# weiaicunzai/pytorch-camvid

Hardware: AMD Instinct MI355X
Metric: images/sec fwd+bwd UNet 3x360x480 bs=8 (higher is better)
Workload: dtype f32; 1 GPU; UNET(3,12) train fwd+bwd+CE, per-GPU batch 8 x 3x360x480 fp32 (BASELINE.json configs[1]); global_batch=8, parallelism=dp1

## Files before the change

### include/cvk.h

```cpp
#ifndef CVK_H
#define CVK_H

#include <stddef.h>
#include <stdint.h>

#ifdef __cplusplus
extern "C" {
#endif

#define CVK_VERSION 100
#define CVK_OK 0
#define CVK_EINVAL (-1)
#define CVK_EWORKSPACE (-2)
#define CVK_STAT_ROWS 64

typedef struct cvk_view {
    float*  ptr;
    int64_t sN, sY, sX;
} cvk_view;

typedef struct cvk_viewh {
    void*   ptr;
    int64_t sN, sY, sX;
} cvk_viewh;
// ... 122 lines not shown
int cvk_conv3x3_thin_fwd(const float* x, const float* w, const float* bias, float* y, float* stats, float* counts, int N, int H,
                         int W, int Cin_ld, int Cout, int ldy, void* stream);
int cvk_thin_wgrad_supported(int Cin, int Cin_ld, int Cout, int ld_dy);
size_t cvk_conv3x3_thin_wgrad_workspace_bytes(int N, int H, int W, int Cin_ld, int Cout);
int cvk_conv3x3_thin_wgrad(const float* x, const float* dy, float* dw, int N, int H, int W, int Cin, int Cin_ld, int Cout,
                           int ld_dy, void* workspace, size_t workspace_bytes, void* stream);

size_t cvk_conv3x3_wgradp_workspace_bytes(int N, int H, int W, int Cin_pad, int Cout);
int cvk_conv3x3_wgradp(const float* x, const float* dy, const float* E6_pre, float* dw, int N, int H, int W, int Cin, int Cin_pad,
                       int Cout, int ld_dy, void* workspace, size_t workspace_bytes, void* stream);
long cvk_wgradp_plane_rows(int N, int H, int W);
int cvk_wgradp_planes(const float* t, int ld, float* planes, int N, int H, int W, int C, int is_dy, void* stream);
size_t cvk_wgradp_gemm_workspace_bytes(int N, int H, int W, int Cin_pad, int Cout);
int cvk_wgradp_gemm(const float* E6, const float* V6, float* dw, int N, int H, int W, int Cin, int Cin_pad, int Cout, void* workspace,
                    size_t workspace_bytes, void* stream);
int cvk_wgradp_zero_pads(float* planes, int N, int H, int W, int C, void* stream);
int cvk_wgradp_zero_pads_sm(float* planes, int N, int H, int W, int C, void* stream);
int cvk_wgradp_planes_sm(const float* x, int ld, float* planes, int N, int H, int W, int C, void* stream);
int cvk_wgradp_gemm_sm(const float* E6, const float* V6sm, float* dw, int N, int H, int W, int Cin, int Cin_pad, int Cout, void* workspace,
                       size_t workspace_bytes, void* stream);
int cvk_wgradp_zero_pads4(float* planes, int N, int H, int W, int C, void* stream);
int cvk_bn_bwd_dx_e4p(cvk_view dout, const float* y, int ldy, const float* scale, const float* shift, const float* mean,
                      const float* rstd, const float* dgamma, const float* dbeta, float* dy, int ld_dy, float* E4p, float* part,
                      int N, int H, int W, int C, int use_batch_stats, void* stream);
int cvk_wgradp_dy_slack(int W);
int cvk_wgradp_gemm_sm_dy(const float* E4p, const float* dy, const float* V6sm, float* dw, int N, int H, int W, int Cin, int Cin_pad, int Cout,
                          void* workspace, size_t workspace_bytes, void* stream);
int cvk_wgradp_gemm_wg(const float* E6, const float* V6, float* dw, int N, int H, int W, int Cin, int Cin_pad, int Cout, void* workspace,
                       size_t workspace_bytes, int max_workgroups, void* stream);
int cvk_wgradp_gemm_sm_wg(const float* E6, const float* V6sm, float* dw, int N, int H, int W, int Cin, int Cin_pad, int Cout, void* workspace,
                          size_t workspace_bytes, int max_workgroups, void* stream);
int cvk_wgradp_gemm_sm_dy_wg(const float* E4p, const float* dy, const float* V6sm, float* dw, int N, int H, int W, int Cin, int Cin_pad, int Cout,
                             void* workspace, size_t workspace_bytes, int max_workgroups, void* stream);
void* cvk_side_begin(void* main_stream);
int cvk_side_join(void* main_stream);
long cvk_side_launches(void);
int cvk_bn_bwd_dx_e6(cvk_view dout, const float* y, int ldy, const float* scale, const float* shift, const float* mean,
                     const float* rstd, const float* dgamma, const float* dbeta, float* dy, int ld_dy, float* E6, float* part,
                     int N, int H, int W, int C, int use_batch_stats, void* stream);

size_t cvk_conv3x3_wgrad_wino4_workspace_bytes(int N, int H, int W, int Cin_pad, int Cout, int ld_dy);
int cvk_conv3x3_wgrad_wino4(const float* x, const float* dy, const float* E_pre, float* dw, int N, int H, int W, int Cin,
                            int Cin_pad, int Cout, int ld_dy, void* workspace, size_t workspace_bytes, void* stream);
int cvk_bn_bwd_e_blocks(int N, int H, int W);
int cvk_bn_bwd_dx_e(cvk_view dout, const float* y, int ldy, const float* scale, const float* shift, const float* mean,
                    const float* rstd, const float* dgamma, const float* dbeta, float* dy, int ld_dy, float* E, float* part,
                    int N, int H, int W, int C, int use_batch_stats, void* stream);

size_t cvk_conv3x3_wgrad_wino_workspace_bytes(int N, int H, int W, int Cin_pad, int Cout);
int cvk_conv3x3_wgrad_wino(const float* x, const float* dy, float* dw, int N, int H, int W, int Cin, int Cin_pad,
                           int Cout, int ld_dy, void* workspace, size_t workspace_bytes, void* stream);

size_t cvk_bn_finalize_workspace_bytes(int P, int C);
int cvk_bn_finalize(const float* stats, int P, int M, int C, const float* gamma, const float* beta,
                    float* mean, float* rstd, float* scale, float* shift,
                    float* running_mean, float* running_var, int64_t* num_batches_tracked,
                    float momentum, float eps, void* workspace, size_t workspace_bytes, void* stream);
int cvk_bn_eval_params(const float* gamma, const float* beta, const float* running_mean, const float* running_var,
                       float* mean, float* rstd, float* scale, float* shift, int C, float eps, void* stream);
int cvk_bn_relu_apply(const float* y, int ldy, const float* scale, const float* shift, cvk_view out,
                      int N, int H, int W, int C, void* stream);
int cvk_bn_relu_apply_pool(const float* y, int ldy, const float* scale, const float* shift, cvk_view out, float* pool,
                           unsigned char* code, int N, int H, int W, int C, void* stream);
int cvk_bn_bwd_blocks(int M);
int cvk_bn_bwd_reduce(cvk_view dout, const float* y, int ldy, const float* scale, const float* shift,
                      const float* mean, const float* rstd, float* part, int N, int H, int W, int C, void* stream);
int cvk_colsum_finalize(const float* part, int PB, int C, float* out0, float* out1, void* stream);
#define CVK_COLSUM_BATCH_MAX 64
typedef struct cvk_colsum_job { const float* part; float* out; int PB, C; } cvk_colsum_job;
int cvk_colsum_finalize_batch(const cvk_colsum_job* jobs, int n, void* stream);
int cvk_bn_relu_apply_amax(const float* y, int ldy, const float* scale, const float* shift, cvk_view out, int N, int H, int W, int C,
                           void* amax_block, void* stream);
int cvk_bn_relu_apply_pool_amax(const float* y, int ldy, const float* scale, const float* shift, cvk_view out, float* pool,
                                unsigned char* code, int N, int H, int W, int C, void* amax_out, void* amax_pool, void* stream);
int cvk_bn_bwd_dx_e_amax(int six, cvk_view dout, const float* y, int ldy, const float* scale, const float* shift, const float* mean,
                         const float* rstd, const float* dgamma, const float* dbeta, float* dy, int ld_dy, float* E, float* part, int N, int H,
                         int W, int C, int use_batch_stats, void* amax_block, void* stream);
int cvk_bn_bwd_dx_amax(cvk_view dout, const float* y, int ldy, const float* scale, const float* shift, const float* mean,
                       const float* rstd, const float* dgamma, const float* dbeta, float* dy, int ld_dy, float* dbias_part, int N,
                       int H, int W, int C, int use_batch_stats, void* amax_block, void* stream);
int cvk_bn_bwd_dx(cvk_view dout, const float* y, int ldy, const float* scale, const float* shift,
                  const float* mean, const float* rstd, const float* dgamma, const float* dbeta,
                  float* dy, int ld_dy, float* dbias_part, int N, int H, int W, int C, int use_batch_stats, void* stream);

int cvk_maxpool2x2_fwd(cvk_view x, float* out, uint8_t* code, int N, int H, int W, int C, void* stream);
int cvk_maxpool2x2_bwd(const float* dout, cvk_view x, const uint8_t* code, cvk_view dx, int accumulate,
                       int N, int H, int W, int C, void* stream);
int cvk_maxpool2x2_bwd_bnred_blocks(int N, int H, int W, int C);
int cvk_maxpool2x2_bwd_bnred(const float* dout, cvk_view x, const uint8_t* code, cvk_view dx, int accumulate, int N, int H, int W, int C,
                             const float* yP, int ldp, const float* scale, const float* shift, const float* mean, const float* rstd,
                             float* part, void* stream);
int cvk_maxunpool2x2_fwd(const float* v, const uint8_t* code, float* out, int N, int H, int W, int C, void* stream);
int cvk_maxunpool2x2_bwd(const float* dout, const uint8_t* code, float* dv, int N, int H, int W, int C, void* stream);
int cvk_pool_code_to_index(const uint8_t* code, int64_t* idx, int N, int H, int W, int C, void* stream);

int cvk_bilinear_up2_fwd(const float* x, float* out, int N, int H, int W, int C, void* stream);
int cvk_bilinear_up2_bwd(const float* dout, float* dx, int N, int H, int W, int C, void* stream);

int cvk_ce_blocks(int M);
int cvk_softmax_ce_fwd(const float* logits, int ld, const int64_t* target, float* part, float* loss,
                       int M, int C, int ignore_index, void* stream);
int cvk_softmax_ce_bwd(const float* logits, int ld, const int64_t* target, const float* loss3, const float* grad_out,
                       float scale, float* dlogits, int ld_d, int M, int C, int ignore_index, void* stream);

#define CVK_REDUCTION_NONE 0
#define CVK_REDUCTION_MEAN 1
#define CVK_REDUCTION_SUM 2
int cvk_ce_ex_part_floats(int M);
int cvk_softmax_ce_fwd_ex(const float* logits, int ld, const int64_t* target, const float* weight, float label_smoothing,
                          int reduction, float* part, float* loss, float* loss_px, int M, int C, int ignore_index, void* stream);
int cvk_softmax_ce_bwd_ex(const float* logits, int ld, const int64_t* target, const float* weight, float label_smoothing,
                          int reduction, const float* loss4, const float* grad_out, float scale, float* dlogits, int ld_d,
                          int M, int C, int ignore_index, void* stream);

#define CVK_DICE_PRESENT 0
#define CVK_DICE_ALL 1
int cvk_seg_loss_part_floats(int M, int C);
int cvk_seg_loss_record_floats(int C);
int cvk_seg_loss_fwd(const float* logits, int ld, const int64_t* target, const float* weight, float ce, float dice, float focal_gamma,
                     float dice_smooth, int dice_average, float* part, float* record, int M, int C, int ignore_index, void* stream);
int cvk_seg_loss_bwd(const float* logits, int ld, const int64_t* target, const float* weight, float ce, float dice, float focal_gamma,
                     const float* record, const float* grad_out, float scale, float* dlogits, int ld_d, int M, int C, int ignore_index,
                     void* stream);

int cvk_kd_loss_part_floats(int M);
int cvk_kd_loss_record_floats(void);
int cvk_kd_loss_fwd(const float* student, int ld_s, const float* teacher, int ld_t, const int64_t* target, const float* weight, float ce,
                    float kd, float tau, float t2, int distill_ignored, float* part, float* record, int M, int C, int ignore_index,
                    void* stream);
int cvk_kd_loss_bwd(const float* student, int ld_s, const float* teacher, int ld_t, const int64_t* target, const float* weight, float ce,
                    float kd, float tau, float t2, int distill_ignored, const float* record, const float* grad_out, float scale,
                    float* dlogits, int ld_d, int M, int C, int ignore_index, void* stream);

int cvk_ohem_scratch_bytes(int M);
int cvk_ohem_record_floats(void);
int cvk_ohem_ce_fwd(const float* logits, int ld, const int64_t* target, const float* weight, float loss_thresh, int min_kept,
                    void* scratch, float* record, float* loss_px, int M, int C, int ignore_index, void* stream);
int cvk_ohem_ce_bwd(const float* logits, int ld, const int64_t* target, const float* weight, const float* record,
                    const float* loss_px, const float* grad_out, float scale, float* dlogits, int ld_d, int M, int C, int ignore_index,
                    void* stream);

#define CVK_LOVASZ_PRESENT 0
#define CVK_LOVASZ_ALL 1
#define CVK_LOVASZ_DIGIT_BITS 8
#define CVK_LOVASZ_SORT_TILE 2048
int64_t cvk_lovasz_workspace_bytes(int M, int C, int segments);
int     cvk_lovasz_record_floats(void);
int64_t cvk_lovasz_sort_dest(int64_t seg_len, int64_t segment, int64_t digit_base, int64_t wg_base, int64_t rank);
int64_t cvk_lovasz_sort_count_index(int64_t work_groups, int64_t segment, int64_t digit, int64_t work_group);
int cvk_lovasz_softmax_fwd(const float* logits, int ld, const int64_t* target, const float* weight, float lovasz, float ce,
                           int classes_mode, int per_image, int N, int pixels_per_image, void* workspace, float* record, float* gmap,
                           int ld_g, int C, int ignore_index, void* stream);
int cvk_lovasz_softmax_bwd(const float* logits, int ld, const int64_t* target, const float* weight, float lovasz, float ce,
                           int per_image, int N, int pixels_per_image, const void* workspace, const float* record, const float* gmap,
                           int ld_g, const float* grad_out, float scale, float* dlogits, int ld_d, int C, int ignore_index,
                           void* stream);

int64_t cvk_edt_workspace_bytes(int N, int H, int W, int num_classes);
int cvk_edt_squared(const int64_t* labels, int N, int H, int W, int num_classes, int ignore_index, void* workspace, int32_t* to_class,
                    int32_t* to_other, void* stream);
int cvk_edt_signed(const int64_t* labels, int N, int H, int W, int num_classes, int ignore_index, void* workspace, float* phi,
                   void* stream);
int cvk_boundary_loss_part_floats(int M, int C);
int cvk_boundary_loss_record_floats(void);
int cvk_boundary_loss_fwd(const float* logits, int ld, const int64_t* target, const float* phi, const float* weight, const float* coef,
                          int want_boundary, int want_ce, unsigned class_mask, float* part, float* record, int M, int C,
// ... 208 lines not shown
```

### pytorch-camvid_amd/_lib.py

```python
import ctypes
import os
import subprocess
import threading

_HERE = os.path.dirname(os.path.abspath(__file__))
LIB_PATH = os.environ.get("CVK_LIB_PATH") or os.path.join(_HERE, "lib", "libcvk.so")
CSRC = os.path.join(_HERE, "csrc")
HEADER = os.path.join(os.path.dirname(_HERE), "include", "cvk.h")

CVK_STAT_ROWS = 64

c_f32p = ctypes.c_void_p
c_i64 = ctypes.c_int64
c_int = ctypes.c_int
c_size = ctypes.c_size_t
c_float = ctypes.c_float
c_vp = ctypes.c_void_p


class View(ctypes.Structure):
    _fields_ = [("ptr", ctypes.c_void_p), ("sN", ctypes.c_int64), ("sY", ctypes.c_int64), ("sX", ctypes.c_int64)]


class ViewH(ctypes.Structure):
# ... 62 lines not shown
    "cvk_side_begin": (c_vp, [c_vp]),
    "cvk_side_join": (c_int, [c_vp]),
    "cvk_side_launches": (ctypes.c_long, []),
    "cvk_conv3x3_wino4f_vplanes": (c_int, [c_vp, c_vp, c_vp, c_vp, c_vp, c_vp, c_vp, c_int, c_int, c_int, c_int, c_int, c_int, c_int, c_vp]),
    "cvk_bn_bwd_dx_e6": (c_int, [View, c_vp, c_int, c_vp, c_vp, c_vp, c_vp, c_vp, c_vp, c_vp, c_int, c_vp, c_vp,
                                 c_int, c_int, c_int, c_int, c_int, c_vp]),
    "cvk_w2d_tiles": (c_int, [c_int, c_int, c_int]),
    "cvk_w6_tiles": (c_int, [c_int, c_int, c_int]),
    "cvk_w6_stat_partials": (c_int, [c_int, c_int, c_int]),
    "cvk_conv3x3_w6_workspace_bytes": (c_size, [c_int, c_int, c_int, c_int, c_int]),
    "cvk_w6_weight_transform": (c_int, [c_vp, c_vp, c_int, c_int, c_vp]),
    "cvk_w6_weight_transform_dgrad": (c_int, [c_vp, c_vp, c_int, c_int, c_vp]),
    "cvk_w6_input_transform": (c_int, [c_vp, c_vp, c_int, c_int, c_int, c_int, c_vp]),
    "cvk_w6_gemm": (c_int, [c_vp, c_vp, c_vp, c_int, c_int, c_int, c_vp]),
    "cvk_w6_wgrad_ksplit": (c_int, [c_int, c_int, c_int]),
    "cvk_w6_dy_transform": (c_int, [c_vp, c_int, c_vp, c_int, c_int, c_int, c_int, c_vp]),
    "cvk_w6_gemm_tn": (c_int, [c_vp, c_vp, c_vp, c_int, c_int, c_int, c_vp]),
    "cvk_w6_wgrad_output": (c_int, [c_vp, c_vp, c_int, c_int, c_int, c_int, c_vp]),
    "cvk_w6_ksplit": (c_int, [c_int, c_int, c_int]),
    "cvk_w6_output": (c_int, [c_vp, c_vp, c_vp, c_vp, c_vp, c_int, c_int, c_int, c_int, c_int, c_int, c_vp]),
    "cvk_w2d_stat_partials": (c_int, [c_int, c_int, c_int]),
    "cvk_conv3x3_w2d_workspace_bytes": (c_size, [c_int, c_int, c_int, c_int, c_int]),
    "cvk_w2d_weight_transform": (c_int, [c_vp, c_vp, c_int, c_int, c_vp]),
    "cvk_w2d_weight_transform_dgrad": (c_int, [c_vp, c_vp, c_int, c_int, c_vp]),
    "cvk_w2d_input_transform": (c_int, [c_vp, c_vp, c_int, c_int, c_int, c_int, c_vp]),
    "cvk_w2d_gemm": (c_int, [c_vp, c_vp, c_vp, c_int, c_int, c_int, c_vp]),
    "cvk_conv3x3_wgrad_w2d_workspace_bytes": (c_size, [c_int, c_int, c_int, c_int, c_int]),
    "cvk_conv3x3_wgrad_w2d": (c_int, [c_vp, c_vp, c_vp, c_int, c_int, c_int, c_int, c_int, c_int, c_int, c_vp, c_size, c_vp]),
    "cvk_w2d_tpad": (c_int, [c_int]),
    "cvk_split3_rows_pad": (c_int, [c_int, c_int]),
    "cvk_split3_planes": (c_int, [c_vp, c_vp, c_int, c_int, c_int, c_int, c_vp]),
    "cvk_w2d_gemm_split3": (c_int, [c_vp, c_vp, c_vp, c_int, c_int, c_int, c_int, c_int, c_int, c_vp]),
    "cvk_w2d_input_transform_split3": (c_int, [c_int, c_vp, c_vp, c_int, c_int, c_int, c_int, c_vp]),
    "cvk_w2d_dy_transform_both_split3": (c_int, [c_int, c_vp, c_int, c_vp, c_vp, c_int, c_int, c_int, c_int, c_int, c_vp]),
    "cvk_w2d_weight_transform_split3": (c_int, [c_int, c_vp, c_vp, c_vp, c_int, c_int, c_int, c_vp]),
    "cvk_w2d_output_plain": (c_int, [c_int, c_vp, c_vp, c_vp, c_vp, c_vp, c_int, c_int, c_int, c_int, c_int, c_vp]),
    "cvk_w2d_gemm_tn_split3_ksplit": (c_int, [c_int, c_int, c_int, c_int]),
    "cvk_w2d_gemm_tn_split3": (c_int, [c_vp, c_vp, c_vp, c_int, c_int, c_int, c_int, c_vp]),
    "cvk_amax_block_words": (c_int, []),
    "cvk_amax_block_value": (ctypes.c_uint, [c_vp, c_int]),
    "cvk_absmax_f32": (c_int, [c_vp, ctypes.c_long, c_int, c_int, c_vp, c_vp]),
    "cvk_split_scale_exponent": (c_int, [c_int, c_int, c_int, ctypes.c_uint]),
    "cvk_split_planes": (c_int, [c_int, c_int, c_int, c_vp, c_vp, c_vp, c_int, c_int, c_int, c_int, c_vp]),
    "cvk_w2d_gemm_split": (c_int, [c_int, c_int, c_vp, c_vp, c_vp, c_vp, c_vp, c_int, c_int, c_int, c_int, c_int, c_int, c_vp]),
    "cvk_w2d_input_transform_split": (c_int, [c_int, c_int, c_vp, c_vp, c_vp, c_int, c_int, c_int, c_int, c_vp]),
    "cvk_w2d_dy_transform_both_split": (c_int, [c_int, c_int, c_vp, c_int, c_vp, c_vp, c_int, c_vp, c_int, c_int, c_int, c_int, c_vp]),
    "cvk_w2d_weight_transform_split": (c_int, [c_int, c_int, c_vp, c_vp, c_vp, c_int, c_int, c_int, c_vp]),
    "cvk_w2d_gemm_tn_split": (c_int, [c_int, c_int, c_vp, c_vp, c_vp, c_vp, c_vp, c_int, c_int, c_int, c_int, c_vp]),
    "cvk_w2d_wgrad_output_f": (c_int, [c_int, c_vp, c_vp, c_int, c_int, c_int, c_int, c_vp]),
    "cvk_w2d_wgrad_ksplit": (c_int, [c_int, c_int, c_int]),
    "cvk_w2d_dy_transform": (c_int, [c_vp, c_int, c_vp, c_int, c_int, c_int, c_int, c_vp]),
    "cvk_w2d_dy_transform_both": (c_int, [c_vp, c_int, c_vp, c_vp, c_int, c_int, c_int, c_int, c_vp]),
    "cvk_w6_dy_transform_both": (c_int, [c_vp, c_int, c_vp, c_vp, c_int, c_int, c_int, c_int, c_vp]),
    "cvk_w2d_gemm_tn": (c_int, [c_vp, c_vp, c_vp, c_int, c_int, c_int, c_vp]),
    "cvk_w2d_wgrad_output": (c_int, [c_vp, c_vp, c_int, c_int, c_int, c_int, c_vp]),
    "cvk_w2d_ksplit": (c_int, [c_int, c_int, c_int]),
    "cvk_w2d_output": (c_int, [c_vp, c_vp, c_vp, c_vp, c_vp, c_int, c_int, c_int, c_int, c_int, c_int, c_vp]),
    "cvk_conv3x3_w2d": (c_int, [c_vp, c_vp, c_vp, c_vp, c_vp, c_vp, c_int, c_int, c_int, c_int, c_int, c_int, c_vp, c_size, c_vp]),
    "cvk_conv3x3_wgrad_wino4_workspace_bytes": (c_size, [c_int, c_int, c_int, c_int, c_int, c_int]),
    "cvk_conv3x3_wgrad_wino4": (c_int, [c_vp, c_vp, c_vp, c_vp, c_int, c_int, c_int, c_int, c_int, c_int, c_int, c_vp, c_size, c_vp]),
    "cvk_bn_bwd_e_blocks": (c_int, [c_int, c_int, c_int]),
    "cvk_bn_bwd_dx_e": (c_int, [View, c_vp, c_int, c_vp, c_vp, c_vp, c_vp, c_vp, c_vp, c_vp, c_int, c_vp, c_vp,
                                c_int, c_int, c_int, c_int, c_int, c_vp]),
    "cvk_conv3x3_wgrad_wino_workspace_bytes": (c_size, [c_int, c_int, c_int, c_int, c_int]),
    "cvk_conv3x3_wgrad_wino": (c_int, [c_vp, c_vp, c_vp, c_int, c_int, c_int, c_int, c_int, c_int, c_int, c_vp, c_size, c_vp]),
    "cvk_bn_finalize_workspace_bytes": (c_size, [c_int, c_int]),
    "cvk_bn_finalize": (c_int, [c_vp, c_int, c_int, c_int, c_vp, c_vp, c_vp, c_vp, c_vp, c_vp, c_vp, c_vp, c_vp,
                                c_float, c_float, c_vp, c_size, c_vp]),
    "cvk_bn_eval_params": (c_int, [c_vp, c_vp, c_vp, c_vp, c_vp, c_vp, c_vp, c_vp, c_int, c_float, c_vp]),
    "cvk_bn_relu_apply": (c_int, [c_vp, c_int, c_vp, c_vp, View, c_int, c_int, c_int, c_int, c_vp]),
    "cvk_bn_relu_apply_pool": (c_int, [c_vp, c_int, c_vp, c_vp, View, c_vp, c_vp, c_int, c_int, c_int, c_int, c_vp]),
    "cvk_bn_bwd_blocks": (c_int, [c_int]),
    "cvk_bn_bwd_reduce": (c_int, [View, c_vp, c_int, c_vp, c_vp, c_vp, c_vp, c_vp, c_int, c_int, c_int, c_int, c_vp]),
    "cvk_colsum_finalize": (c_int, [c_vp, c_int, c_int, c_vp, c_vp, c_vp]),
    "cvk_colsum_finalize_batch": (c_int, [c_vp, c_int, c_vp]),
    "cvk_bn_bwd_dx": (c_int, [View, c_vp, c_int, c_vp, c_vp, c_vp, c_vp, c_vp, c_vp, c_vp, c_int, c_vp,
                              c_int, c_int, c_int, c_int, c_int, c_vp]),
    "cvk_bn_relu_apply_amax": (c_int, [c_vp, c_int, c_vp, c_vp, View, c_int, c_int, c_int, c_int, c_vp, c_vp]),
    "cvk_bn_relu_apply_pool_amax": (c_int, [c_vp, c_int, c_vp, c_vp, View, c_vp, c_vp, c_int, c_int, c_int, c_int, c_vp, c_vp, c_vp]),
    "cvk_bn_bwd_dx_e_amax": (c_int, [c_int, View, c_vp, c_int, c_vp, c_vp, c_vp, c_vp, c_vp, c_vp, c_vp, c_int, c_vp, c_vp,
                                     c_int, c_int, c_int, c_int, c_int, c_vp, c_vp]),
    "cvk_bn_bwd_dx_amax": (c_int, [View, c_vp, c_int, c_vp, c_vp, c_vp, c_vp, c_vp, c_vp, c_vp, c_int, c_vp,
                                   c_int, c_int, c_int, c_int, c_int, c_vp, c_vp]),
    "cvk_maxpool2x2_fwd": (c_int, [View, c_vp, c_vp, c_int, c_int, c_int, c_int, c_vp]),
    "cvk_maxpool2x2_bwd": (c_int, [c_vp, View, c_vp, View, c_int, c_int, c_int, c_int, c_int, c_vp]),
    "cvk_maxpool2x2_bwd_bnred_blocks": (c_int, [c_int, c_int, c_int, c_int]),
    "cvk_maxpool2x2_bwd_bnred": (c_int, [c_vp, View, c_vp, View, c_int, c_int, c_int, c_int, c_int, c_vp, c_int, c_vp, c_vp, c_vp, c_vp, c_vp, c_vp]),
    "cvk_maxunpool2x2_fwd": (c_int, [c_vp, c_vp, c_vp, c_int, c_int, c_int, c_int, c_vp]),
    "cvk_maxunpool2x2_bwd": (c_int, [c_vp, c_vp, c_vp, c_int, c_int, c_int, c_int, c_vp]),
    "cvk_pool_code_to_index": (c_int, [c_vp, c_vp, c_int, c_int, c_int, c_int, c_vp]),
    "cvk_bilinear_up2_fwd": (c_int, [c_vp, c_vp, c_int, c_int, c_int, c_int, c_vp]),
    "cvk_bilinear_up2_bwd": (c_int, [c_vp, c_vp, c_int, c_int, c_int, c_int, c_vp]),
    "cvk_ce_blocks": (c_int, [c_int]),
    "cvk_softmax_ce_fwd": (c_int, [c_vp, c_int, c_vp, c_vp, c_vp, c_int, c_int, c_int, c_vp]),
    "cvk_softmax_ce_bwd": (c_int, [c_vp, c_int, c_vp, c_vp, c_vp, c_float, c_vp, c_int, c_int, c_int, c_int, c_vp]),
    "cvk_ce_ex_part_floats": (c_int, [c_int]),
    "cvk_softmax_ce_fwd_ex": (c_int, [c_vp, c_int, c_vp, c_vp, c_float, c_int, c_vp, c_vp, c_vp, c_int, c_int, c_int, c_vp]),
    "cvk_softmax_ce_bwd_ex": (c_int, [c_vp, c_int, c_vp, c_vp, c_float, c_int, c_vp, c_vp, c_float, c_vp, c_int, c_int, c_int, c_int,
                                      c_vp]),
    "cvk_seg_loss_part_floats": (c_int, [c_int, c_int]),
    "cvk_seg_loss_record_floats": (c_int, [c_int]),
    "cvk_seg_loss_fwd": (c_int, [c_vp, c_int, c_vp, c_vp, c_float, c_float, c_float, c_float, c_int, c_vp, c_vp, c_int, c_int, c_int, c_vp]),
    "cvk_seg_loss_bwd": (c_int, [c_vp, c_int, c_vp, c_vp, c_float, c_float, c_float, c_vp, c_vp, c_float, c_vp, c_int, c_int, c_int, c_int,
                                 c_vp]),
    "cvk_kd_loss_part_floats": (c_int, [c_int]),
    "cvk_kd_loss_record_floats": (c_int, []),
    "cvk_kd_loss_fwd": (c_int, [c_vp, c_int, c_vp, c_int, c_vp, c_vp, c_float, c_float, c_float, c_float, c_int, c_vp, c_vp, c_int, c_int,
                                c_int, c_vp]),
    "cvk_kd_loss_bwd": (c_int, [c_vp, c_int, c_vp, c_int, c_vp, c_vp, c_float, c_float, c_float, c_float, c_int, c_vp, c_vp, c_float, c_vp,
                                c_int, c_int, c_int, c_int, c_vp]),
    "cvk_ohem_scratch_bytes": (c_int, [c_int]),
    "cvk_ohem_record_floats": (c_int, []),
    "cvk_ohem_ce_fwd": (c_int, [c_vp, c_int, c_vp, c_vp, c_float, c_int, c_vp, c_vp, c_vp, c_int, c_int, c_int, c_vp]),
    "cvk_ohem_ce_bwd": (c_int, [c_vp, c_int, c_vp, c_vp, c_vp, c_vp, c_vp, c_float, c_vp, c_int, c_int, c_int, c_int, c_vp]),
    "cvk_lovasz_workspace_bytes": (ctypes.c_int64, [c_int, c_int, c_int]),
    "cvk_lovasz_record_floats": (c_int, []),
    "cvk_lovasz_sort_dest": (ctypes.c_int64, [ctypes.c_int64] * 5),
    "cvk_lovasz_sort_count_index": (ctypes.c_int64, [ctypes.c_int64] * 4),
    "cvk_lovasz_softmax_fwd": (c_int, [c_vp, c_int, c_vp, c_vp, c_float, c_float, c_int, c_int, c_int, c_int, c_vp, c_vp, c_vp, c_int,
                                       c_int, c_int, c_vp]),
    "cvk_lovasz_softmax_bwd": (c_int, [c_vp, c_int, c_vp, c_vp, c_float, c_float, c_int, c_int, c_int, c_vp, c_vp, c_vp, c_int, c_vp,
                                       c_float, c_vp, c_int, c_int, c_int, c_vp]),
    "cvk_edt_workspace_bytes": (ctypes.c_int64, [c_int, c_int, c_int, c_int]),
    "cvk_edt_squared": (c_int, [c_vp, c_int, c_int, c_int, c_int, c_int, c_vp, c_vp, c_vp, c_vp]),
    "cvk_edt_signed": (c_int, [c_vp, c_int, c_int, c_int, c_int, c_int, c_vp, c_vp, c_vp]),
    "cvk_boundary_loss_part_floats": (c_int, [c_int, c_int]),
    "cvk_boundary_loss_record_floats": (c_int, []),
    "cvk_boundary_loss_fwd": (c_int, [c_vp, c_int, c_vp, c_vp, c_vp, c_vp, c_int, c_int, ctypes.c_uint, c_vp, c_vp, c_int, c_int, c_int,
                                      c_vp]),
    "cvk_boundary_loss_bwd": (c_int, [c_vp, c_int, c_vp, c_vp, c_vp, c_int, c_int, ctypes.c_uint, c_vp, c_vp, c_float, c_vp, c_int, c_int,
                                      c_int, c_int, c_vp]),
    "cvk_class_histogram": (c_int, [c_vp, c_int, c_int, c_i64, c_int, c_int, c_vp, c_vp]),
    "cvk_argmax_channels": (c_int, [c_vp, c_int, c_vp, c_int, c_int, c_vp]),
    "cvk_confusion_accumulate": (c_int, [c_vp, c_vp, c_vp, c_int, c_int, c_int, c_vp]),
    "cvk_boundary_counts": (c_int, [c_vp, c_vp, c_vp, c_int, c_int, c_int, c_int, c_int, c_int, c_vp]),
    "cvk_boundary_map": (c_int, [c_vp, c_vp, c_vp, c_int, c_int, c_int, c_int, c_int, c_vp]),
    "cvk_surface_workspace_bytes": (ctypes.c_int64, [c_int, c_int, c_int, c_int]),
    "cvk_surface_record_slots": (c_int, []),
    "cvk_surface_distances": (c_int, [c_vp, c_vp, c_int, c_int, c_int, c_int, c_int, c_int, c_int, c_vp, c_vp, c_vp, c_vp]),
    "cvk_cheb_workspace_bytes": (ctypes.c_int64, [c_int, c_int, c_int]),
    "cvk_cheb_depth": (c_int, [c_vp, c_vp, c_vp, c_vp, c_vp, c_int, c_int, c_int, c_int, c_int, c_int, c_int, c_vp]),
    "cvk_boundary_iou_counts": (c_int, [c_vp, c_vp, c_vp, c_vp, c_vp, c_vp, c_vp, c_int, c_int, c_int, c_int, c_int, c_int, c_vp]),
    "cvk_cc_workspace_bytes": (ctypes.c_int64, [c_int, c_int, c_int, c_int]),
    "cvk_cc_record_slots": (c_int, []),
    "cvk_cc_label": (c_int, [c_vp, c_vp, c_vp, c_int, c_int, c_int, c_int, c_int, c_int, c_vp, c_vp]),
    "cvk_cc_filter": (c_int, [c_vp, c_vp, c_vp, c_vp, c_vp, c_int, c_int, c_int, c_int, c_int, c_int, c_int, c_int, c_i64, c_vp, c_vp]),
    "cvk_crf_tile": (c_int, [c_int, c_int, c_int, c_vp, c_vp, c_vp]),
    "cvk_crf_step": (c_int, [c_vp, c_int, c_int, c_vp, c_vp, c_vp, c_vp, c_int, c_i64, c_i64, c_i64, c_i64, c_vp, c_vp, c_vp, c_vp, c_float,
                             c_float, c_float, c_vp, c_int, c_int, c_int, c_int, c_int, c_int, c_int, c_int, c_vp]),
    "cvk_calib_accumulate": (c_int, [c_vp, c_int, c_vp, c_vp, c_vp, c_vp, c_vp, c_vp, c_vp, c_int, c_int, c_int, c_int, c_vp]),
    "cvk_calib_newton_accumulate": (c_int, [c_vp, c_int, c_vp, c_vp, c_vp, c_int, c_int, c_int, c_vp]),
    "cvk_calib_newton_step": (c_int, [c_vp, c_vp, c_int, c_int, c_vp]),
    "cvk_tta_accumulate": (c_int, [c_vp, c_int, c_int, c_int, c_vp, c_vp, c_int, c_int, c_int, c_int, c_int, c_int, c_int, c_float, c_vp]),
    "cvk_tta_resize_input": (c_int, [c_vp, c_i64, c_i64, c_i64, c_i64, c_vp, c_int, c_int, c_int, c_int, c_int, c_int, c_vp]),
    "cvk_window_merge": (c_int, [c_vp, c_int, c_vp, c_vp, c_int, c_int, c_int, c_int, c_int, c_int, c_int, c_int, c_int, c_int, c_vp]),
    "cvk_preprocess_u8": (c_int, [c_vp, c_vp, c_int, c_int, c_int, ctypes.POINTER(ctypes.c_float), ctypes.POINTER(ctypes.c_float), c_vp]),
    "cvk_augment_record_bytes": (c_int, []),
    "cvk_augment_u8": (c_int, [c_vp, c_vp, c_int, c_int, c_int, c_int, c_int, c_int, c_vp, ctypes.POINTER(ctypes.c_float),
                               ctypes.POINTER(ctypes.c_float), c_vp, c_vp, c_vp, c_vp]),
    "cvk_crop_record_bytes": (c_int, []),
    "cvk_crop_select": (c_int, [c_vp, c_int, c_int, c_int, c_int, c_int, c_int, c_vp, c_int, ctypes.c_double, c_vp, c_vp, c_vp]),
    "cvk_crop_augment_u8": (c_int, [c_vp, c_vp, c_int, c_int, c_int, c_int, c_int, c_int, c_vp, c_vp, ctypes.POINTER(ctypes.c_float),
                                    ctypes.POINTER(ctypes.c_float), c_i64, c_int, c_vp, c_vp, c_vp, c_vp]),
    "cvk_bf16s_rows_pad": (c_int, [c_int]),
    "cvk_bf16s_stat_partials": (c_int, [c_int, c_int, c_int]),
    "cvk_bf16s_stat_partials_c": (c_int, [c_int, c_int, c_int, c_int, c_int]),
# ... 170 lines not shown
```

### pytorch-camvid_amd/conv_bf16.py

```python
import torch

from ._lib import check
from .conv_fp32 import ConvBnRelu
from .engine import _BF16, _F32, _empty, _timed, channels_last


def bf16_kernel_name(lib, N, H, W, cin_ld, cout, stats):
    k = lib.cvk_conv3x3_bf16s_kernel(N, H, W, cin_ld, cout, 1 if stats else 0)
    st = "true" if stats else "false"
    if k == 1:
        return f"k_conv_bf16q<{st}>"
    if k in (2, 3):
        return f"k_conv_bf16h<{st}, 0, {'true' if k == 3 else 'false'}>"
    if k in (4, 5):
        return f"k_conv_bf16s_strip<{1 if cin_ld == 32 else 2}, {st}>" + (" x2" if k == 5 else "")
    return f"k_conv_bf16s<{128 if cout > 64 else 64}, {st}>"


class ConvBnReluBf16(ConvBnRelu):
    _pitch, _ydt = staticmethod(int), _BF16
    _BN = ("cvk_bn_bwd_blocks_bf16", "cvk_bn_bwd_reduce_bf16", "k_bnbwd_bf16<reduce>")

    def thin_mode(self, R, dgrad, ld_dy=0):
        if not R.thin or self.src.H * self.src.W * max(self.src.ld, self.cout, ld_dy, 64) * 2 >= 2 ** 31:
            return 0
        if dgrad:
            return R.lib.cvk_thin_bf16_mode(self.cin, self.cout, ld_dy, self.src.ld, 1) if self.src.ld == 64 and self.cin == 64 else 0
        return R.lib.cvk_thin_bf16_mode(self.cin, self.cout, self.src.ld, self.cout, 0)

    def packs_wanted(self, R, need_grad):
        want = []
        if not self.thin_mode(R, False):
            want.append((((self.pslot, "f"), "bf16"), 0, self.cout, self.src.ld))
        if need_grad and self.src_needs_grad and not self.thin_mode(R, True, max(32, self.cout)):
            want.append((((self.pslot, "d"), "bf16"), 1, self.cin, max(32, self.cout)))
        return want

    def _pack(self, R, st, w, side, mode, kpad):
        lib, s, dev, wc = R.lib, st.stream, st.device, channels_last(w)

        def build_thin():
            t = torch.empty(lib.cvk_thin_bf16_pack_elems(mode), device=dev, dtype=_BF16)
            check(lib.cvk_pack_weight_thin_bf16(wc.data_ptr(), t.data_ptr(), self.cout, self.cin, mode, s), "cvk_pack_weight_thin_bf16")
            return t

        def build():
            fn = "cvk_pack_weight_%s_bf16" % ("fwd" if side == "f" else "dgrad")
            t = torch.empty(lib.cvk_bf16s_rows_pad(self.cout if side == "f" else self.cin) * 9 * kpad, device=dev, dtype=_BF16)
            check(getattr(lib, fn)(wc.data_ptr(), t.data_ptr(), self.cout, self.cin, kpad, s), fn)
            return t
        return R.derived(((self.pslot, side), "thinb"), w, build_thin) if mode else R.derived(((self.pslot, side), "bf16"), w, build)

    def _weight_fwd(self, R, st, w):
        if self.cout % 4:
            raise NotImplementedError("bf16 mode needs output channel counts that are multiples of 4")
        tmode = self.thin_mode(R, False)
        return tmode, self._pack(R, st, w, "f", tmode, self.src.ld)

    def _stat_partials(self, R, wk):
        src = self.src
        P = R.lib.cvk_thin_bf16_stat_partials(src.N, src.H, src.W) if wk[0] else R.lib.cvk_bf16s_stat_partials_c(src.N, src.H, src.W, src.ld, self.cout)
        return P, P

    def _conv(self, R, st, rt, X, wk, b, y, stats, P):
        lib, s, src, C, (tmode, wb) = R.lib, st.stream, self.src, self.cout, wk
        N, H, W, M = src.N, src.H, src.W, src.M
        flops = 18.0 * M * C * self.cin
        sp = stats.data_ptr() if stats is not None else None
        cnt = sp + 4 * 2 * P * C if stats is not None else None
        if tmode:
            _timed(R, {1: "k_thinb_head_fwd", 2: "k_thinb_wide<1>"}.get(tmode), flops, lambda: check(
                lib.cvk_conv3x3_thin_bf16(X.data_ptr(), wb.data_ptr(), b.data_ptr(), y.data_ptr(), sp, cnt, N, H, W, src.ld, C, C,
                                          tmode, s), "cvk_conv3x3_thin_bf16"), nbytes=2.0 * M * (src.ld + C))
        elif stats is not None:
            _timed(R, bf16_kernel_name(lib, N, H, W, src.ld, C, True), flops, lambda: check(
                lib.cvk_conv3x3_bf16s_wg(X.data_ptr(), wb.data_ptr(), b.data_ptr(), y.data_ptr(), sp, cnt, N, H, W, src.ld, C, C,
                                         R.launch_wgs(), s), "cvk_conv3x3_bf16s"))
        else:
            _timed(R, bf16_kernel_name(lib, N, H, W, src.ld, C, False), flops, lambda: check(
                lib.cvk_conv3x3_bf16s(X.data_ptr(), wb.data_ptr(), b.data_ptr(), y.data_ptr(), None, None, N, H, W, src.ld, C, C, s), "cvk_conv3x3_bf16s"))
        return ((P, cnt) if stats is not None else None), None

    def _bn_apply(self, R, st, y, psc, psh):
        src, dst, C = self.src, self.dst, self.cout
        out = R.alloc_act(st, dst.buf, st.device)
        out_f32 = 1 if dst.buf.dtype == _F32 else 0
        pool = R.alloc_act(st, self.pool_dst, st.device) if self.pool_dst is not None else None
        nbytes = (2.0 + (4.0 if out_f32 else 2.0)) * src.M * C + (0.5 * src.M * C if pool is not None else 0.0)
        _timed(R, "k_apply_bf16" + ("<pool>" if pool is not None else ""), nbytes, lambda: check(
            R.lib.cvk_bn_relu_apply_bf16(y.data_ptr(), C, psc, psh, dst.hview(out), out_f32, pool.data_ptr() if pool is not None else None,
                                         src.N, src.H, src.W, C, st.stream), "cvk_bn_relu_apply_bf16"), "byte")

    def _dout(self, st):
        return self.dst.hview(st.grad[self.dst.buf.id]), 1 if self.dst.buf.dtype == _F32 else 0

    def _bn_bwd(self, R, st, rt, bn, gg, gbe, part, PB, gb):
        src, C, ld_dy = self.src, self.cout, max(32, self.cout)
        dy = torch.empty(src.M * ld_dy, device=st.device, dtype=_BF16)
        _timed(R, "k_bnbwd_bf16<dx>", ((4.0 if bn[1] else 2.0) + 4.0) * src.M * C, lambda: check(
            R.lib.cvk_bn_bwd_dx_bf16(*bn, gg, gbe, dy.data_ptr(), ld_dy, part.data_ptr(),
                                     src.N, src.H, src.W, C, 1 if self.bn_train else 0, st.stream), "cvk_bn_bwd_dx_bf16"), "byte")
        if gb is not None:
            R.defer_colsum(st, part, PB, C, gb)
        return dy, None, None

    def _data_grad(self, R, st, rt, dy, Vb, am_dy):
        lib, s, src, C, ld_dy = R.lib, st.stream, self.src, self.cout, max(32, self.cout)
        N, H, W, M = src.N, src.H, src.W, src.M
        flops = 18.0 * M * C * self.cin
        if src.id in st.grad:
            raise NotImplementedError("conv data-grad must be the first writer of its input's gradient buffer")
        dmode = self.thin_mode(R, True, ld_dy)
        dX = torch.empty((N, H, W, src.ld), device=st.device, dtype=_BF16)
        wd = self._pack(R, st, st.params[4 * self.pslot], "d", dmode, ld_dy)
        if dmode:
            _timed(R, "k_thinb_wide<3>(dgrad)", flops, lambda: check(
                lib.cvk_conv3x3_thin_bf16(dy.data_ptr(), wd.data_ptr(), None, dX.data_ptr(), None, None, N, H, W, ld_dy, C, src.ld, dmode, s),
                "cvk_conv3x3_thin_bf16(dgrad)"), nbytes=2.0 * M * (ld_dy + src.ld))
        else:
            _timed(R, bf16_kernel_name(lib, N, H, W, ld_dy, self.cin, False), flops, lambda: check(
                lib.cvk_conv3x3_bf16s_wg(dy.data_ptr(), wd.data_ptr(), None, dX.data_ptr(), None, None, N, H, W, ld_dy, self.cin, src.ld,
                                         R.launch_wgs(), s), "cvk_conv3x3_bf16s(dgrad)"))
        st.grad[src.id] = dX

    def _weight_grad(self, R, st, saved, dy, gw, E, Eb, am_dy):
        lib, src, C = R.lib, self.src, self.cout
        N, H, W = src.N, src.H, src.W
        S = lib.cvk_conv3x3_wgrad_bf16s_splits(N, H, W, self.cin, C)
        n = C * 9 * self.cin
        slab = None if S == 1 else _empty(S * n, st.device)
        _timed(R, "k_wgrad_bf16r", 18.0 * src.M * C * self.cin, lambda: check(
            lib.cvk_conv3x3_wgrad_bf16s_slabs(st.act[src.id].data_ptr(), dy.data_ptr(), gw if slab is None else slab.data_ptr(), N, H, W, self.cin,
                                              src.ld, C, max(32, C), 4 * S * n, st.stream), "cvk_conv3x3_wgrad_bf16s_slabs"))
        if slab is not None:
            R.defer_wreduce(st, slab, S, n, gw)
```

### pytorch-camvid_amd/conv_fp32.py

```python
import torch

from . import _lib
from ._lib import check
from .engine import _BF16, _F32, Op, Saved, _empty, _timed, amax_blocks, channels_last
from .route import pad4


def w2fn(lib, tile, name):
    return getattr(lib, ("cvk_w6_" if tile == 6 else "cvk_w2d_") + name)


_PLANE_DT = {0: _F32, 2: torch.float16, 3: _BF16}


def planes2d(lib, tile, N, H, W, fmt=0):
    T = w2fn(lib, tile, "tiles")(N, H, W)
    return 64 if tile == 6 else 36, T, lib.cvk_split3_rows_pad(T, 256) if fmt else lib.cvk_w2d_tpad(T)


def plane_elems(NX, Tp, C, fmt=0):
    return NX * (C // 32) * fmt * Tp * 32 if fmt else NX * Tp * C + 128


def absmax(R, t, rows, cols, ld, s, what):
# ... 219 lines not shown
                w2fn(lib, tile, "input_transform")(x.data_ptr(), V.data_ptr(), N, H, W, k_ch, s), "cvk_w2d_input_transform(wgrad)"), "byte")
        ws = R.workspace(4 * ((0 if Eb is not None else efl) + f * NX * C * k_ch), x.device)
        Ep, Pp = (Eb.data_ptr(), ws.data_ptr()) if Eb is not None else (ws.data_ptr(), ws.data_ptr() + 4 * efl)
        if Eb is None:
            _timed(R, "k_w2d_dy", 4.0 * (M + NX * T) * C, lambda: check(
                w2fn(lib, tile, "dy_transform")(dy.data_ptr(), ldy, Ep, N, H, W, C, s), "cvk_w2d_dy_transform"), "byte")
        _timed(R, "k_w2d_gemm_tn", self.flops, lambda: check(
            w2fn(lib, tile, "gemm_tn")(Ep, V.data_ptr(), Pp, T, k_ch, C, s), "cvk_w2d_gemm_tn"), executed=2.0 * NX * Tp * k_ch * C)
        _timed(R, "k_w2d_wgrad_out", 4.0 * (NX * f + 9) * C * self.cin, lambda: check(
            w2fn(lib, tile, "wgrad_output")(Pp, self.gw, T, self.cin, k_ch, C, s), "cvk_w2d_wgrad_output"), "byte")

    def w2d_split(self, tile, fmt, V, am_v, Eb, am_dy):
        R, lib, s, k_ch, C = self.R, self.lib, self.s, self.k_ch, self.cout
        NX, _, Tp = planes2d(lib, tile, self.N, self.H, self.W, fmt)
        f = lib.cvk_w2d_gemm_tn_split3_ksplit(NX, Tp, k_ch, C)
        ws = R.workspace(4 * f * NX * C * k_ch, self.x.device)
        _timed(R, "k_gemm_tn_" + ("split3" if fmt == 3 else "split2h"), self.flops, lambda: check(
            lib.cvk_w2d_gemm_tn_split(fmt, tile, Eb.data_ptr(), V.data_ptr(), ws.data_ptr(), am_dy.data_ptr() if am_dy is not None else None,
                                      am_v.data_ptr() if am_v is not None else None, NX, Tp, k_ch, C, s), "cvk_w2d_gemm_tn_split"),
            executed=2.0 * (6 if fmt == 3 else 3) * NX * Tp * k_ch * C)
        _timed(R, "k_w2d_wgrad_out", 4.0 * (NX * f + 9) * C * self.cin, lambda: check(
            lib.cvk_w2d_wgrad_output_f(tile, ws.data_ptr(), self.gw, self.cin, k_ch, C, f, s), "cvk_w2d_wgrad_output_f"), "byte")

    def wgradp(self, own_v, V, E, sm_dy):
        R, lib, s, x, dy = self.R, self.lib, self.s, self.x, self.dy
        N, H, W, M, k_ch, C, ldy = self.N, self.H, self.W, self.M, self.k_ch, self.cout, self.ldy
        rows6 = lib.cvk_wgradp_plane_rows(N, H, W)
        wsb = lib.cvk_wgradp_gemm_workspace_bytes(N, H, W, k_ch, C)
        nE = 0 if E is not None else 6 * rows6 * C
        nV = 6 * rows6 * k_ch if own_v else 0
        ws = R.workspace(4 * (nV + nE) + wsb, x.device)
        V6p = ws.data_ptr() if own_v else V.data_ptr()
        E6p = E.data_ptr() if E is not None else ws.data_ptr() + 4 * nV
        slabp = ws.data_ptr() + 4 * (nV + nE)
        if own_v:
            _timed(R, "k_wgradp_planes", 4.0 * (M + 6.0 * rows6) * k_ch, lambda: check(
                lib.cvk_wgradp_planes(x.data_ptr(), k_ch, V6p, N, H, W, k_ch, 0, s), "cvk_wgradp_planes(x)"), "byte")
        if E is None:
            _timed(R, "k_wgradp_planes", 4.0 * (M + 6.0 * rows6) * C, lambda: check(
                lib.cvk_wgradp_planes(dy.data_ptr(), ldy, E6p, N, H, W, C, 1, s), "cvk_wgradp_planes(dy)"), "byte")
        fn = "cvk_wgradp_gemm_sm_dy" if sm_dy else ("cvk_wgradp_gemm" if own_v else "cvk_wgradp_gemm_sm")
        ev = (E6p, dy.data_ptr(), V6p) if sm_dy else (E6p, V6p)
        _timed(R, "k_wgradp_gemm", self.flops, lambda: check(getattr(lib, fn)(*ev, self.gw, N, H, W, self.cin, k_ch, C, slabp, wsb, s), fn),
               executed=9.0 * M * C * self.cin)

    def w4(self, E):
        R, lib, N, H, W, k_ch, C, ldy = self.R, self.lib, self.N, self.H, self.W, self.k_ch, self.cout, self.ldy
        wsb = lib.cvk_conv3x3_wgrad_wino4_workspace_bytes(N, H, W, k_ch, C, ldy)
        ws = R.workspace(wsb, self.x.device)
        _timed(R, f"k_wgrad_wino4<{'128' if C > 64 else '64'}, 128, 2, 2>", self.flops, lambda: check(
            lib.cvk_conv3x3_wgrad_wino4(self.x.data_ptr(), self.dy.data_ptr(), E.data_ptr() if E is not None else None, self.gw, N, H, W,
                                        self.cin, k_ch, C, ldy, ws.data_ptr(), wsb, self.s), "cvk_conv3x3_wgrad_wino4"))

    def direct(self, fam):
        R, lib, N, H, W, M, k_ch, C, ldy = self.R, self.lib, self.N, self.H, self.W, self.M, self.k_ch, self.cout, self.ldy
        fn = {"thin": "cvk_conv3x3_thin_wgrad", "w2": "cvk_conv3x3_wgrad_wino", "direct": "cvk_conv3x3_wgrad"}[fam]
        wsb = getattr(lib, fn + "_workspace_bytes")(N, H, W, k_ch, C)
        ws = R.workspace(wsb, self.x.device)
        head = k_ch == 64
        name, kw = {"thin": ("k_thin_co_wgrad" if head else "k_thin_ci_wgrad",
                             dict(executed=18.0 * M * (16 * self.cin if head else C * 16 / 3.0), nbytes=4.0 * M * (k_ch + ldy))),
                    "w2": (f"k_wgrad_wino<{'128' if C > 64 else '64'}, 128, 2, 2>", {}), "direct": (conv_kernel_name("wgrad", C, k_ch), {})}[fam]
        _timed(R, name, self.flops, lambda: check(getattr(lib, fn)(
            self.x.data_ptr(), self.dy.data_ptr(), self.gw, N, H, W, self.cin, k_ch, C, ldy, ws.data_ptr(), wsb, self.s), fn), **kw)


def conv_kernel_name(kind, n_cols, k_ch=32):
    if kind in ("wino4", "wino"):
        return "k_conv3x3_%s<%s>" % (kind, "128, 128, 2, 2" if n_cols > 64 else ("128, 64, 2, 2" if n_cols > 32 else "128, 32, 4, 1"))
    if kind == "wgrad":
        if n_cols <= 16 and k_ch == 64:
            return "k_wgrad_smallco"
        t = "128, 128, 2, 2" if n_cols > 64 else ("64, 128, 2, 2" if n_cols > 32 else "32, 256, 1, 4")
        if 32 < n_cols <= 64 and k_ch * 9 <= 64:
            t = "64, 64, 2, 2"
        return f"k_conv3x3_wgrad<{t}>"
    t = "128, 128, 2, 2" if n_cols > 64 else ("128, 64, 2, 2" if n_cols > 32 else "256, 32, 4, 1")
    return f"k_conv3x3_igemm<{t}, {'true' if kind == 'fwd' else 'false'}, {'true' if k_ch % 32 == 0 else 'false'}>"


class ConvBnRelu(Op):
    _pitch, _ydt = staticmethod(pad4), _F32
    _BN = ("cvk_bn_bwd_blocks", "cvk_bn_bwd_reduce", "k_bn_bwd<reduce>")

    def __init__(self, src, dst, pslot, holder, cin, cout, src_needs_grad, bn_train=True, req=(True, True, True, True)):
        self.src, self.dst, self.pslot, self.holder = src, dst, pslot, holder
        self.cin, self.cout, self.src_needs_grad = cin, cout, src_needs_grad
        self.bn_train = bool(bn_train)
        self.w_req, self.b_req, self.g_req, self.be_req = (bool(r) for r in req)
        self.name = None
        self.pool_dst = None
        self.pool_op = None
        assert src.C == cin and dst.C == cout and dst.H == src.H and dst.W == src.W

    @property
    def trainable(self):
        return self.w_req or self.b_req or self.g_req or self.be_req

    @property
    def active(self):
        return self.trainable or self.src_needs_grad

    @property
    def label(self):
        return self.name or "conv block #%d" % self.pslot

    def _grad_targets(self, R, st, ld):
        gw, gb, gg, gbe = R.grad_ptrs(st, self.pslot)
        if not (self.g_req and self.be_req):
            sc = _empty(2 * ld, st.device)
            st.scratch.append(sc)
            gg = gg if self.g_req else sc.data_ptr()
            gbe = gbe if self.be_req else sc.data_ptr() + 4 * ld
        return (gw if self.w_req else None), (gb if self.b_req else None), gg, gbe

    def _weight_fwd(self, R, st, w):
        ldx, wc = self.src.ld, channels_last(w)
        if ldx == self.cin and wc is w:
            return w
        def build():
            out = _empty(self.cout * 9 * ldx, w.device)
            check(R.lib.cvk_pack_weight_fwd(wc.data_ptr(), out.data_ptr(), self.cout, self.cin, ldx, st.stream), "cvk_pack_weight_fwd")
            return out
        return R.derived(((self.pslot, "f"), "pack"), w, build)

    def _stat_partials(self, R, wk):
        lib, src = R.lib, self.src
        P = (src.M + _lib.CVK_STAT_ROWS - 1) // _lib.CVK_STAT_ROWS
        return P, max(P, lib.cvk_w2d_stat_partials(src.N, src.H, src.W), lib.cvk_w6_stat_partials(src.N, src.H, src.W),
                      lib.cvk_thin_stat_partials(src.N, src.H, src.W, src.ld))

    def _conv(self, R, st, rt, X, wk, b, y, stats, P):
        lib, s, src = R.lib, st.stream, self.src
        N, H, W, M, C, ldy = src.N, src.H, src.W, src.M, self.cout, pad4(self.cout)
        sp = stats.data_ptr() if stats is not None else None
        flops = 18.0 * M * C * self.cin
        if rt.fwd == "thin":
            Pt = lib.cvk_thin_stat_partials(N, H, W, src.ld)
            cnt = sp + 4 * 2 * Pt * C if sp is not None else None
            head = src.ld == 64
            _timed(R, "k_thin_co_fwd" if head else "k_thin_ci_fwd", flops, lambda: check(
                lib.cvk_conv3x3_thin_fwd(X.data_ptr(), wk.data_ptr(), b.data_ptr(), y.data_ptr(), sp, cnt, N, H, W, src.ld, C, ldy, s),
                "cvk_conv3x3_thin_fwd"), executed=18.0 * M * (16 * self.cin if head else C * src.ld), nbytes=4.0 * M * (src.ld + ldy))
            return ((Pt, cnt) if sp is not None else None), None
        if rt.fwd == "direct":
            _timed(R, conv_kernel_name("fwd", ldy, src.ld), flops, lambda: check(
                lib.cvk_conv3x3_fwd(X.data_ptr(), wk.data_ptr(), b.data_ptr(), y.data_ptr(), sp, N, H, W, src.ld, C, ldy, s), "cvk_conv3x3_fwd"))
            return None, None
        c = WinoConv(R, s, X, wk, b.data_ptr(), y, sp, N, H, W, src.ld, C, ldy, flops, st.params[4 * self.pslot], (self.pslot, "f"))
        counted = c.run(rt.fwd, rt.tile, rt.split, keep=rt.keeps_v, x_amax=st.amax.get(src.id))
        return counted, ((c.v, c.v_amax) if rt.keeps_v else None)

    def _bn_params(self, R, st, stats, counted, P, Pw, gamma, beta, ptrs):
        lib, C, bn = R.lib, self.cout, self.holder.conv_bn()[1]
        if stats is None:
            return check(lib.cvk_bn_eval_params(gamma.data_ptr(), beta.data_ptr(), bn.running_mean.data_ptr(), bn.running_var.data_ptr(), *ptrs, C,
                                                float(bn.eps), st.stream), "cvk_bn_eval_params")
        wsb = lib.cvk_bn_finalize_workspace_bytes(Pw, C)
        ws = R.workspace(wsb, st.device)
        track = bn.track_running_stats and bn.running_mean is not None
        mom = 0.1 if bn.momentum is None else float(bn.momentum)
        tail = (self.src.M, C, gamma.data_ptr(), beta.data_ptr(), *ptrs, bn.running_mean.data_ptr() if track else None,
                bn.running_var.data_ptr() if track else None, bn.num_batches_tracked.data_ptr() if track else None,
                mom, float(bn.eps), ws.data_ptr(), wsb, st.stream)
        if counted is None:
            check(lib.cvk_bn_finalize(stats.data_ptr(), P, *tail), "cvk_bn_finalize")
        else:
            check(lib.cvk_bn_finalize_counts(stats.data_ptr(), counted[1], counted[0], *tail), "cvk_bn_finalize_counts")

    def _bn_apply(self, R, st, y, psc, psh):
        lib, s, src, dst = R.lib, st.stream, self.src, self.dst
        N, H, W, M, C, ldy, dev = src.N, src.H, src.W, src.M, self.cout, pad4(self.cout), st.device
        out = R.alloc_act(st, dst.buf, dev)
        pooled = False
        if self.pool_dst is not None and C % 4 == 0:
            pool = R.alloc_act(st, self.pool_dst, dev)
            code = torch.empty(self.pool_dst.M * self.pool_dst.ld, device=dev, dtype=torch.uint8) if self.pool_op.keep_code else None
            ap = st.amax.get(self.pool_dst.id)
            rc = _timed(R, "k_bn_relu_apply<pool>", (8.0 + 1.0 + (0.25 if code is not None else 0.0)) * M * C, lambda: amax_call(
                lib, "cvk_bn_relu_apply_pool", (y.data_ptr(), ldy, psc, psh, dst.cview(out), pool.data_ptr(), code.data_ptr() if code is not None else None,
                                                N, H, W, C), (st.amax.get(dst.buf.id), ap), s), "byte")
            pooled = rc == 0
            if not pooled and ap is not None:
                st.amax.pop(self.pool_dst.id)
            if pooled and code is not None:
                st.saved[self.pool_op.idx] = code
        st.pooled_by_block[self.idx] = pooled
        if not pooled:
            _timed(R, "k_bn_relu_apply", 8.0 * M * C, lambda: check(amax_call(
                lib, "cvk_bn_relu_apply", (y.data_ptr(), ldy, psc, psh, dst.cview(out), N, H, W, C), (st.amax.get(dst.buf.id),), s), "cvk_bn_relu_apply"), "byte")

    def fwd(self, R, st):
        src, C, ld, dev = self.src, self.cout, self._pitch(self.cout), st.device
        rt = st.routes[self.idx] if st.routes is not None else None
        w, b, gamma, beta = st.params[4 * self.pslot:4 * self.pslot + 4]
        wk = self._weight_fwd(R, st, w)
        y = torch.empty(src.M * ld, device=dev, dtype=self._ydt)
        bnp = _empty(4 * ld, dev)
        ptrs = tuple(bnp.data_ptr() + 4 * ld * i for i in range(4))
        stats, P, Pw = None, 0, 0
        if self.bn_train:
            if src.M <= 1:
                raise ValueError(f"Expected more than 1 value per channel when training, got input size {[src.N, C, src.H, src.W]}")
            P, Pw = self._stat_partials(R, wk)
            stats = _empty(2 * Pw * C + Pw, dev)
        counted, kept = self._conv(R, st, rt, st.act[src.id], wk, b, y, stats, P)
        self._bn_params(R, st, stats, counted, P, Pw, gamma, beta, ptrs)
        self._bn_apply(R, st, y, ptrs[2], ptrs[3])
        if st.need_grad and self.active:
            st.saved[self.idx] = Saved(y, bnp, rt, kept)

    def _bn_sums(self, R, st, bn, gg, gbe):
        lib, s, src, C, (blocks, fn, name) = R.lib, st.stream, self.src, self.cout, self._BN
        PB = getattr(lib, blocks)(src.M)
        part = _empty(2 * PB * C, st.device)
        pre = st.bnred.pop(self.idx, None)
        if pre is not None:
            check(lib.cvk_colsum_finalize(pre[0].data_ptr(), pre[1], C, gbe, gg, s), "cvk_colsum_finalize")
        elif self.bn_train or self.g_req or self.be_req:
            _timed(R, name, float(self.dst.buf.esize + self._ydt.itemsize) * src.M * C, lambda: check(
                getattr(lib, fn)(*bn, part.data_ptr(), src.N, src.H, src.W, C, s), fn), "byte")
            check(lib.cvk_colsum_finalize(part.data_ptr(), PB, C, gbe, gg, s), "cvk_colsum_finalize")
        if self.w_req or self.b_req or self.src_needs_grad:
            return part, PB
        R.grads_ready(st, self.pslot)
        return None

    _BN_E = {"dx+E": (0, "cvk_bn_bwd_dx_e", 16.0), "dx+E6": (1, "cvk_bn_bwd_dx_e6", 24.0), "dx+E4p": (2, "cvk_bn_bwd_dx_e4p", 16.0)}

    def _bn_bwd(self, R, st, rt, bn, gg, gbe, part, PB, gb):
        lib, s, src, kind = R.lib, st.stream, self.src, rt.bn_bwd
        N, H, W, M, C, ldy = src.N, src.H, src.W, src.M, self.cout, pad4(self.cout)
        if kind == "dx+E4p":
            dyb = _empty(M * ldy + lib.cvk_wgradp_dy_slack(W) * ldy, st.device)
            dyb[M * ldy:].zero_()
            dy = dyb[:M * ldy]
        else:
            dy = torch.zeros(M * ldy, device=st.device, dtype=_F32) if ldy != C else _empty(M * ldy, st.device)
        want_amax = rt.dy_amax and bool(st.amax_spare)
        head, tail = (*bn, gg, gbe, dy.data_ptr(), ldy), (part.data_ptr(), N, H, W, C, 1 if self.bn_train else 0)
        if kind != "dx":
            mode, plain, eb = self._BN_E[kind]
            if kind == "dx+E":
                E = _empty(4 * N * H * ((W + 3) // 4) * ldy, st.device)
            else:
                E = _empty((4 if mode == 2 else 6) * lib.cvk_wgradp_plane_rows(N, H, W) * C, st.device)
                check((lib.cvk_wgradp_zero_pads4 if mode == 2 else lib.cvk_wgradp_zero_pads)(E.data_ptr(), N, H, W, C, s), "cvk_wgradp_zero_pads")
            blk = st.amax_spare[-1] if want_amax else None
            rc = _timed(R, "k_bn_bwd<%s>" % kind, (12.0 * M + eb * N * H * ((W + 3) // 4)) * C, lambda: (
                lib.cvk_bn_bwd_dx_e_amax(mode, *head, E.data_ptr(), *tail, blk.data_ptr(), s) if blk is not None
                else getattr(lib, plain)(*head, E.data_ptr(), *tail, s)), "byte")
            if rc == 0:
                if gb is not None:
                    R.defer_colsum(st, part, lib.cvk_bn_bwd_e_blocks(N, H, W), C, gb)
                return dy, E, (st.amax_spare.pop() if blk is not None else None)
        am = st.amax_spare.pop() if want_amax else None
        _timed(R, "k_bn_bwd<dx>", 12.0 * M * C, lambda: check(amax_call(lib, "cvk_bn_bwd_dx", (*head, *tail), (am,), s), "cvk_bn_bwd_dx"), "byte")
        if gb is not None:
            R.defer_colsum(st, part, PB, C, gb)
        return dy, None, am

    def _dy_both(self, R, st, rt, dy, am_dy):
        if rt is None or not rt.dy_both:
            return None, None, am_dy
        lib, s, src = R.lib, st.stream, self.src
        N, H, W, M, C, ldy = src.N, src.H, src.W, src.M, self.cout, pad4(self.cout)
        tile, fmt = rt.tile, rt.split
        NX, T, Tp = planes2d(lib, tile, N, H, W, fmt)
        Eb, Vb = (torch.empty(plane_elems(NX, Tp, C, fmt), device=st.device, dtype=_PLANE_DT[fmt]) for _ in range(2))
        if fmt:
            if fmt == 2 and am_dy is None:
                am_dy = absmax(R, dy, M, C, ldy, s, "dy")
            _timed(R, "k_w2d_dy<both,%s>" % ("split3" if fmt == 3 else "split2h"), (4.0 * M + 4.0 * fmt * NX * T) * C, lambda: check(
                lib.cvk_w2d_dy_transform_both_split(fmt, tile, dy.data_ptr(), ldy, Vb.data_ptr(), Eb.data_ptr(), 1,
                                                    am_dy.data_ptr() if am_dy is not None else None, N, H, W, C, s), "cvk_w2d_dy_transform_both_split"), "byte")
        else:
            _timed(R, "k_w2d_dy<both>", 4.0 * (M + 2 * NX * T) * C, lambda: check(
                w2fn(lib, tile, "dy_transform_both")(dy.data_ptr(), ldy, Vb.data_ptr(), Eb.data_ptr(), N, H, W, C, s), "cvk_w2d_dy_transform_both"), "byte")
        return Eb, Vb, am_dy

    def _data_grad(self, R, st, rt, dy, Vb, am_dy):
        lib, s, src = R.lib, st.stream, self.src
        N, H, W, M, C, ldy, dev = src.N, src.H, src.W, src.M, self.cout, pad4(self.cout), st.device
        flops = 18.0 * M * C * self.cin
        if src.id in st.grad:
            raise NotImplementedError("conv data-grad must be the first writer of its input's gradient buffer")
        R.side_join(st)
        w = st.params[4 * self.pslot]
        wc = channels_last(w)

        def packed():
            wd_ = _empty(src.ld * 9 * ldy, dev)
            _timed(R, "k_pack_weight_dgrad", 4.0 * 9 * (C * self.cin + src.ld * ldy), lambda: check(
                lib.cvk_pack_weight_dgrad(wc.data_ptr(), wd_.data_ptr(), C, self.cin, src.ld, ldy, s), "cvk_pack_weight_dgrad"), "byte")
            return wd_
        dX = _empty(M * src.ld, dev).view(N, H, W, src.ld)
        wd = R.derived(((self.pslot, "d"), "pack"), w, packed) if rt.dgrad in ("thin", "direct") else None
        if rt.dgrad == "thin":
            _timed(R, "k_thin_ci_fwd(dgrad)", flops, lambda: check(
                lib.cvk_conv3x3_thin_fwd(dy.data_ptr(), wd.data_ptr(), None, dX.data_ptr(), None, None, N, H, W, ldy, src.ld, src.ld, s),
                "cvk_conv3x3_thin_fwd(dgrad)"), executed=18.0 * M * ldy * src.ld, nbytes=4.0 * M * (src.ld + ldy))
        elif rt.dgrad == "direct":
            _timed(R, conv_kernel_name("dgrad", src.ld, ldy), flops, lambda: check(
                lib.cvk_conv3x3_fwd(dy.data_ptr(), wd.data_ptr(), None, dX.data_ptr(), None, N, H, W, ldy, src.ld, src.ld, s), "cvk_conv3x3_fwd(dgrad)"))
        else:
            prod = st.plan.sole_producer(src) if rt.dgrad_bnred else None
            bnred = None
            if prod is not None and prod.bn_train and prod.idx in st.saved and pad4(prod.cout) == prod.cout == src.ld:
                bnred = st.saved[prod.idx].pointers(src.ld)
            c = WinoConv(R, s, dy, packed, None, dX, None, N, H, W, ldy, src.ld, src.ld, flops, w, (self.pslot, "d"), "(dgrad)", dgrad_of=(wc, C, self.cin))
            c.run(rt.dgrad, rt.dgrad_tile, rt.split, v_pre=Vb, x_amax=am_dy, bnred=bnred)
            if c.bnred_sums is not None:
                st.bnred[prod.idx] = c.bnred_sums
        st.grad[src.id] = dX

    def _dout(self, st):
        return (self.dst.cview(st.grad[self.dst.buf.id]),)

    def _weight_grad(self, R, st, saved, dy, gw, E, Eb, am_dy):
        src, rt, s = self.src, saved.rt, st.stream
        x = st.act[src.id]
        side = st.side and rt.wgrad in R.side_families
        if side:
            s = R.side_begin(st, x, dy, E, Eb, am_dy, saved)
        else:
            R.side_join(st)
        wg = WeightGrad(R, s, x, dy, gw, src.N, src.H, src.W, self.cin, src.ld, self.cout, pad4(self.cout), 18.0 * src.M * self.cout * self.cin)
        wg.run(rt.wgrad, rt.tile, rt.split, *(saved.kept or (None, None)), E, rt.bn_bwd == "dx+E4p", Eb, am_dy)
        if side:
            st.side_keep.extend(wg.keep)
            st.side_keep.append(R.workspace(0, x.device))

    def bwd(self, R, st):
        saved = st.saved.pop(self.idx, None)
        if not self.active:
            return
        rt, ld = saved.rt, self._pitch(self.cout)
        gw, gb, gg, gbe = self._grad_targets(R, st, ld)
        yp, *bnp = saved.pointers(ld)
        bn = (*self._dout(st), yp, ld, *bnp)
# ... 11 lines not shown
```

### pytorch-camvid_amd/csrc/bn.hip

```cpp
#include "cvk_common.h"

namespace {

__global__ __launch_bounds__(256) void k_bn_stats_l1(const float* __restrict__ stats, double* __restrict__ ws, int P, int M,
                                                    int C, int rows_per_g) {
    __shared__ double red[3][4][64];
    const int c = blockIdx.x * 64 + (threadIdx.x & 63);
    const int g = threadIdx.x >> 6;
    const int pbeg = blockIdx.y * rows_per_g, pend = min(P, pbeg + rows_per_g);
    double a = 0.0, b = 0.0, q = 0.0;
    if (c < C) {
        const double inv_full = 1.0 / (double)CVK_STAT_ROWS;
        const int last = P - 1;
        const double inv_last = 1.0 / (double)(M - last * CVK_STAT_ROWS);
        double a1 = 0.0, b1 = 0.0, q1 = 0.0;
        int p = pbeg + g;
        for (; p + 4 < pend; p += 8) {
            const double s0 = stats[(size_t)p * C + c], s1 = stats[(size_t)(p + 4) * C + c];
            const double m0 = stats[(size_t)(P + p) * C + c], m1 = stats[(size_t)(P + p + 4) * C + c];
            a += s0; b += m0; q += s0 * s0 * (p == last ? inv_last : inv_full);
            a1 += s1; b1 += m1; q1 += s1 * s1 * (p + 4 == last ? inv_last : inv_full);
        }
        for (; p < pend; p += 4) {
            const double s0 = stats[(size_t)p * C + c];
            a += s0; b += stats[(size_t)(P + p) * C + c]; q += s0 * s0 * (p == last ? inv_last : inv_full);
        }
        a += a1; b += b1; q += q1;
    }
    red[0][g][threadIdx.x & 63] = a;
    red[1][g][threadIdx.x & 63] = b;
    red[2][g][threadIdx.x & 63] = q;
    __syncthreads();
    if (g == 0 && c < C) {
        const int l = threadIdx.x;
        double* o = ws + ((size_t)blockIdx.y * C + c) * 3;
        o[0] = (red[0][0][l] + red[0][1][l]) + (red[0][2][l] + red[0][3][l]);
        o[1] = (red[1][0][l] + red[1][1][l]) + (red[1][2][l] + red[1][3][l]);
        o[2] = (red[2][0][l] + red[2][1][l]) + (red[2][2][l] + red[2][3][l]);
    }
}

__global__ __launch_bounds__(256) void k_bn_stats_l1_counts(const float* __restrict__ stats, const float* __restrict__ cnt,
                                                           double* __restrict__ ws, int P, int C, int rows_per_g) {
    __shared__ double red[3][4][64];
    const int c = blockIdx.x * 64 + (threadIdx.x & 63);
    const int g = threadIdx.x >> 6;
    const int pbeg = blockIdx.y * rows_per_g, pend = min(P, pbeg + rows_per_g);
    double a = 0.0, b = 0.0, q = 0.0;
    if (c < C)
        for (int p = pbeg + g; p < pend; p += 4) {
            const double s0 = stats[(size_t)p * C + c];
            a += s0;
            b += stats[(size_t)(P + p) * C + c];
            q += s0 * s0 / (double)cnt[p];
        }
    red[0][g][threadIdx.x & 63] = a;
    red[1][g][threadIdx.x & 63] = b;
    red[2][g][threadIdx.x & 63] = q;
    __syncthreads();
    if (g == 0 && c < C) {
        const int l = threadIdx.x;
        double* o = ws + ((size_t)blockIdx.y * C + c) * 3;
        o[0] = (red[0][0][l] + red[0][1][l]) + (red[0][2][l] + red[0][3][l]);
        o[1] = (red[1][0][l] + red[1][1][l]) + (red[1][2][l] + red[1][3][l]);
        o[2] = (red[2][0][l] + red[2][1][l]) + (red[2][2][l] + red[2][3][l]);
    }
}

__global__ __launch_bounds__(256) void k_bn_stats_l2(const double* __restrict__ ws, int G, int M, int C, const float* __restrict__ gamma,
                              const float* __restrict__ beta, float* mean, float* rstd, float* scale, float* shift,
                              float* running_mean, float* running_var, int64_t* nbt, float momentum, float eps) {
    __shared__ double red[3][4][64];
    const int l = threadIdx.x & 63, lane = threadIdx.x >> 6;
    const int c = blockIdx.x * 64 + l;
    if (blockIdx.x == 0 && threadIdx.x == 0 && nbt != nullptr) *nbt += 1;
    double a = 0.0, b = 0.0, q = 0.0;
    if (c < C)
        for (int g = lane; g < G; g += 4) {
            const double* o = ws + ((size_t)g * C + c) * 3;
            a += o[0];
            b += o[1];
            q += o[2];
        }
// ... 67 lines not shown
template <int V>
__global__ __launch_bounds__(256) void k_bn_relu_apply(const float* __restrict__ y, int ldy, const float* __restrict__ scale,
                                                      const float* __restrict__ shift, float* __restrict__ out, PixMap om,
                                                      int M, int C, unsigned* __restrict__ amax) {
    typedef typename Vec<V>::T VT;
    const int cvn = C / V;
    const long total = (long)M * cvn;
    float mx = 0.f;
    const unsigned snap = cvk_amax_snapshot(amax);
    for (long i = (long)blockIdx.x * blockDim.x + threadIdx.x; i < total; i += (long)gridDim.x * blockDim.x) {
        const int m = (int)(i / cvn);
        const int c = (int)(i - (long)m * cvn) * V;
        const VT v = *reinterpret_cast<const VT*>(y + (size_t)m * ldy + c);
        const VT sc = *reinterpret_cast<const VT*>(scale + c);
        const VT sh = *reinterpret_cast<const VT*>(shift + c);
        VT o;
#pragma unroll
        for (int j = 0; j < V; ++j) {
            const float r = fmaxf(vget<V>(v, j) * vget<V>(sc, j) + vget<V>(sh, j), 0.f);
            vset<V>(o, j, r);
            mx = fmaxf(mx, r);
        }
        *reinterpret_cast<VT*>(out + om.off(m) + c) = o;
    }
    if (amax != nullptr) cvk_amax_publish_wg(mx, amax, snap);
}

__global__ __launch_bounds__(256) void k_bn_relu_apply_pool(const float* __restrict__ y, int ldy, const float* __restrict__ scale,
                                                           const float* __restrict__ shift, float* __restrict__ out, PixMap om,
                                                           float* __restrict__ pool, unsigned char* __restrict__ code, int N, int H,
                                                           int W, int C, unsigned* __restrict__ amax_out, unsigned* __restrict__ amax_pool) {
    const int cvn = C >> 2, Hc = (H + 1) >> 1, Wc = (W + 1) >> 1, Ho = H >> 1, Wo = W >> 1;
    const long total = (long)N * Hc * Wc * cvn;
    float mxo = 0.f, mxp = 0.f;
    const unsigned snapo = cvk_amax_snapshot(amax_out), snapp = cvk_amax_snapshot(amax_pool);
    for (long i = (long)blockIdx.x * blockDim.x + threadIdx.x; i < total; i += (long)gridDim.x * blockDim.x) {
        const int cv = (int)(i % cvn);
        long t = i / cvn;
        const int xc = (int)(t % Wc);
        t /= Wc;
        const int yc = (int)(t % Hc), n = (int)(t / Hc);
        const int c = cv * 4;
        const f32x4 sc = *reinterpret_cast<const f32x4*>(scale + c);
        const f32x4 sh = *reinterpret_cast<const f32x4*>(shift + c);
        f32x4 v[4];
#pragma unroll
        for (int k = 0; k < 4; ++k) {
            const int yy = 2 * yc + (k >> 1), xx = 2 * xc + (k & 1);
            if (yy < H && xx < W) {
                const int m = (n * H + yy) * W + xx;
                const f32x4 a = *reinterpret_cast<const f32x4*>(y + (size_t)m * ldy + c);
#pragma unroll
                for (int j = 0; j < 4; ++j) {
                    v[k][j] = fmaxf(a[j] * sc[j] + sh[j], 0.f);
                    mxo = fmaxf(mxo, v[k][j]);
                }
                *reinterpret_cast<f32x4*>(out + om.off(m) + c) = v[k];
            }
        }
        if (yc < Ho && xc < Wo) {
            f32x4 best = v[0];
            unsigned char cd[4] = {0, 0, 0, 0};
#pragma unroll
            for (int k = 1; k < 4; ++k)
#pragma unroll
                for (int j = 0; j < 4; ++j) {
                    const float a = v[k][j], b = best[j];
                    if (a > b || a != a) { best[j] = a; cd[j] = (unsigned char)k; }
                }
            const long o = (((long)n * Ho + yc) * Wo + xc) * C + c;
            *reinterpret_cast<f32x4*>(pool + o) = best;
#pragma unroll
            for (int j = 0; j < 4; ++j) mxp = fmaxf(mxp, best[j]);
            if (code != nullptr) {
#pragma unroll
                for (int j = 0; j < 4; ++j) code[o + j] = cd[j];
            }
        }
    }
    if (amax_out != nullptr) cvk_amax_publish_wg(mxo, amax_out, snapo);
    if (amax_pool != nullptr) { __syncthreads(); cvk_amax_publish_wg(mxp, amax_pool, snapp); }
}

template <int V, int MODE>
__global__ __launch_bounds__(256) void k_bn_bwd(const float* __restrict__ dout, PixMap dm, const float* __restrict__ y, int ldy,
                                               const float* __restrict__ scale, const float* __restrict__ shift,
                                               const float* __restrict__ mean, const float* __restrict__ rstd,
                                               const float* __restrict__ dgamma, const float* __restrict__ dbeta,
                                               float* __restrict__ dy, int ld_dy, float* __restrict__ part, int M, int C,
                                               int rows, int PB, int cchunk, int use_batch_stats, unsigned* __restrict__ amax) {
    typedef typename Vec<V>::T VT;
    __shared__ float red[2][256 * V];
    float mx = 0.f;
    const unsigned snap = MODE == 1 ? cvk_amax_snapshot(amax) : 0u;
    const int c0 = blockIdx.y * cchunk;
    const int cw = min(cchunk, C - c0);
    const int cvn = cw / V;
    const int ppp = 256 / cvn;
    const int t = threadIdx.x;
    const bool active = t < cvn * ppp;
    const int cv = t % cvn, pr = t / cvn;
    const int c = c0 + cv * V;
    const int mbeg = blockIdx.x * rows, mend = min(M, mbeg + rows);

    float s0[V], s1[V];
#pragma unroll
    for (int j = 0; j < V; ++j) { s0[j] = 0.f; s1[j] = 0.f; }
    if (active) {
        const VT sc = *reinterpret_cast<const VT*>(scale + c);
        const VT sh = *reinterpret_cast<const VT*>(shift + c);
        const VT mu = *reinterpret_cast<const VT*>(mean + c);
        const VT rs = *reinterpret_cast<const VT*>(rstd + c);
        float k1[V], k2[V];
        if (MODE == 1) {
            const float invM = 1.f / (float)M;
#pragma unroll
            for (int j = 0; j < V; ++j) {
                k1[j] = use_batch_stats ? dbeta[c + j] * invM : 0.f;
                k2[j] = use_batch_stats ? dgamma[c + j] * invM : 0.f;
            }
        }
#pragma unroll 4
        for (int m = mbeg + pr; m < mend; m += ppp) {
            const VT d = *reinterpret_cast<const VT*>(dout + dm.off(m) + c);
            const VT yy = *reinterpret_cast<const VT*>(y + (size_t)m * ldy + c);
            VT o;
#pragma unroll
            for (int j = 0; j < V; ++j) {
                const float yv = vget<V>(yy, j);
                const float g = (yv * vget<V>(sc, j) + vget<V>(sh, j) > 0.f) ? vget<V>(d, j) : 0.f;
                const float xh = (yv - vget<V>(mu, j)) * vget<V>(rs, j);
                if (MODE == 0) {
                    s0[j] += g;
                    s1[j] += g * xh;
                } else {
                    const float r = vget<V>(sc, j) * (g - k1[j] - xh * k2[j]);
                    vset<V>(o, j, r);
                    s0[j] += r;
                    mx = fmaxf(mx, fabsf(r));
                }
            }
            if (MODE == 1) *reinterpret_cast<VT*>(dy + (size_t)m * ld_dy + c) = o;
        }
    }
    if (MODE == 1 && amax != nullptr) cvk_amax_publish(mx, amax, snap);
    if (part == nullptr) return;
#pragma unroll
    for (int j = 0; j < V; ++j) {
        red[0][t * V + j] = s0[j];
        if (MODE == 0) red[1][t * V + j] = s1[j];
    }
    __syncthreads();
    if (t < cvn) {
#pragma unroll
        for (int j = 0; j < V; ++j) {
            float a = 0.f, b = 0.f;
            for (int p = 0; p < ppp; ++p) {
                a += red[0][(p * cvn + t) * V + j];
                if (MODE == 0) b += red[1][(p * cvn + t) * V + j];
            }
            part[(size_t)blockIdx.x * C + c0 + t * V + j] = a;
            if (MODE == 0) part[(size_t)(PB + blockIdx.x) * C + c0 + t * V + j] = b;
        }
    }
}

__global__ __launch_bounds__(256) void k_bn_bwd_dx_e(const float* __restrict__ dout, PixMap dm, const float* __restrict__ y, int ldy,
                                                    const float* __restrict__ scale, const float* __restrict__ shift,
                                                    const float* __restrict__ mean, const float* __restrict__ rstd,
                                                    const float* __restrict__ dgamma, const float* __restrict__ dbeta,
                                                    float* __restrict__ dy, int ld_dy, float* __restrict__ E,
                                                    float* __restrict__ part, int M, int C, int W, int Wt, int Mt, int tiles,
                                                    int cchunk, int use_batch_stats, int six_H, int six_Wtp, long six_rows,
                                                    unsigned* __restrict__ amax) {
    __shared__ float red[256 * 4];
    float mx = 0.f;
    const unsigned snap = cvk_amax_snapshot(amax);
    const int c0 = blockIdx.y * cchunk;
    const int cw = min(cchunk, C - c0);
    const int cvn = cw / 4;
    const int ppp = 256 / cvn;
    const int t = threadIdx.x;
    const bool active = t < cvn * ppp;
    const int cv = t % cvn, pr = t / cvn;
    const int c = c0 + cv * 4;
    const int tbeg = blockIdx.x * tiles, tend = min(Mt, tbeg + tiles);
    float s0[4] = {0.f, 0.f, 0.f, 0.f};
    if (active) {
        const f32x4 sc = *reinterpret_cast<const f32x4*>(scale + c);
        const f32x4 sh = *reinterpret_cast<const f32x4*>(shift + c);
        const f32x4 mu = *reinterpret_cast<const f32x4*>(mean + c);
        const f32x4 rs = *reinterpret_cast<const f32x4*>(rstd + c);
        f32x4 k1 = {0.f, 0.f, 0.f, 0.f}, k2 = {0.f, 0.f, 0.f, 0.f};
        if (use_batch_stats) {
            const float invM = 1.f / (float)M;
#pragma unroll
            for (int j = 0; j < 4; ++j) { k1[j] = dbeta[c + j] * invM; k2[j] = dgamma[c + j] * invM; }
        }
        const size_t plane = (size_t)Mt * ld_dy;
        for (int tl = tbeg + pr; tl < tend; tl += ppp) {
            const int row = tl / Wt, xt = tl - row * Wt;
            const int m0 = row * W + 4 * xt;
            f32x4 r[4];
#pragma unroll
            for (int i = 0; i < 4; ++i) {
                r[i] = f32x4{0.f, 0.f, 0.f, 0.f};
                if (4 * xt + i < W) {
                    const int m = m0 + i;
                    const f32x4 d = *reinterpret_cast<const f32x4*>(dout + dm.off(m) + c);
                    const f32x4 yy = *reinterpret_cast<const f32x4*>(y + (size_t)m * ldy + c);
#pragma unroll
                    for (int j = 0; j < 4; ++j) {
                        const float g = (yy[j] * sc[j] + sh[j] > 0.f) ? d[j] : 0.f;
                        const float xh = (yy[j] - mu[j]) * rs[j];
                        const float v = sc[j] * (g - k1[j] - xh * k2[j]);
                        r[i][j] = v;
                        s0[j] += v;
                        mx = fmaxf(mx, fabsf(v));
                    }
                    *reinterpret_cast<f32x4*>(dy + (size_t)m * ld_dy + c) = r[i];
                }
            }
            const f32x4 a = r[0] + r[2], b = r[1] + r[3], cc = r[0] + 4.f * r[2], dd = 2.f * r[1] + 8.f * r[3];
            if (six_H == 0) {
                float* o = E + (size_t)tl * ld_dy + c;
                *reinterpret_cast<f32x4*>(o) = a + b;
                *reinterpret_cast<f32x4*>(o + plane) = a - b;
                *reinterpret_cast<f32x4*>(o + 2 * plane) = cc + dd;
                *reinterpret_cast<f32x4*>(o + 3 * plane) = cc - dd;
            } else {
                const int n = row / six_H, yy = row - n * six_H;
                const size_t prow = (size_t)six_Wtp + ((size_t)n * (six_H + 2) + yy + 1) * six_Wtp + xt;
                const size_t ps = (size_t)six_rows * C;
                float* o = E + prow * C + c;
                if (six_rows < 0) {
                    const size_t p4 = (size_t)(-six_rows) * C;
                    *reinterpret_cast<f32x4*>(o) = a + b;
                    *reinterpret_cast<f32x4*>(o + p4) = a - b;
                    *reinterpret_cast<f32x4*>(o + 2 * p4) = cc + dd;
                    *reinterpret_cast<f32x4*>(o + 3 * p4) = cc - dd;
                } else {
                    *reinterpret_cast<f32x4*>(o) = r[0];
                    *reinterpret_cast<f32x4*>(o + ps) = a + b;
                    *reinterpret_cast<f32x4*>(o + 2 * ps) = a - b;
                    *reinterpret_cast<f32x4*>(o + 3 * ps) = cc + dd;
                    *reinterpret_cast<f32x4*>(o + 4 * ps) = cc - dd;
                    *reinterpret_cast<f32x4*>(o + 5 * ps) = r[3];
                }
            }
        }
    }
    if (amax != nullptr) cvk_amax_publish(mx, amax, snap);
    if (part == nullptr) return;
#pragma unroll
    for (int j = 0; j < 4; ++j) red[t * 4 + j] = s0[j];
    __syncthreads();
    if (t < cvn) {
#pragma unroll
        for (int j = 0; j < 4; ++j) {
            float a = 0.f;
            for (int p = 0; p < ppp; ++p) a += red[(p * cvn + t) * 4 + j];
            part[(size_t)blockIdx.x * C + c0 + t * 4 + j] = a;
        }
    }
}

__global__ __launch_bounds__(1024) void k_colsum_finalize(const float* __restrict__ part, int PB, int C, float* out0,
                                                         float* out1) {
    __shared__ double red[16][64];
    const int l = threadIdx.x & 63, g = threadIdx.x >> 6;
    const int c = blockIdx.x * 64 + l;
    const int which = blockIdx.y;
    const float* src = part + (size_t)which * PB * C;
    double a = 0.0;
    if (c < C) {
        double a1 = 0.0, a2 = 0.0, a3 = 0.0;
        int p = g;
        for (; p + 48 < PB; p += 64) {
            a += (double)src[(size_t)p * C + c];
            a1 += (double)src[(size_t)(p + 16) * C + c];
// ... 98 lines not shown
        cvk_set_error("cvk_bn_finalize_counts: workspace too small");
        return CVK_EWORKSPACE;
    }
    const int G = P < 32 ? 1 : (P / 32 < 64 ? P / 32 : 64);
    const int rows_per_g = cvk_cdiv(P, G);
    hipStream_t s = (hipStream_t)stream;
    hipLaunchKernelGGL(k_bn_stats_l1_counts, dim3(cvk_cdiv(C, 64), G), dim3(256), 0, s, stats, counts, (double*)workspace, P, C, rows_per_g);
    hipLaunchKernelGGL(k_bn_stats_l2, dim3(cvk_cdiv(C, 64)), dim3(256), 0, s, (const double*)workspace, G, M, C, gamma, beta, mean,
                       rstd, scale, shift, running_mean, running_var, num_batches_tracked, momentum, eps);
    CVK_LAUNCH_RETURN("cvk_bn_finalize_counts");
}

extern "C" int cvk_bn_eval_params(const float* gamma, const float* beta, const float* running_mean, const float* running_var,
                                  float* mean, float* rstd, float* scale, float* shift, int C, float eps, void* stream) {
    CVK_CHECK_ARG(gamma && beta && running_mean && running_var && mean && rstd && scale && shift && C > 0, "cvk_bn_eval_params: bad arguments");
    hipLaunchKernelGGL(k_bn_eval_params, dim3(cvk_cdiv(C, 256)), dim3(256), 0, (hipStream_t)stream, gamma, beta, running_mean,
                       running_var, mean, rstd, scale, shift, C, eps);
    CVK_LAUNCH_RETURN("cvk_bn_eval_params");
}

static int bn_relu_apply_launch(const char* who, const float* y, int ldy, const float* scale, const float* shift, cvk_view out, int N, int H,
                                int W, int C, void* amax, void* stream);
extern "C" int cvk_bn_relu_apply(const float* y, int ldy, const float* scale, const float* shift, cvk_view out, int N, int H,
                                 int W, int C, void* stream) {
    return bn_relu_apply_launch("cvk_bn_relu_apply", y, ldy, scale, shift, out, N, H, W, C, nullptr, stream);
}
extern "C" int cvk_bn_relu_apply_amax(const float* y, int ldy, const float* scale, const float* shift, cvk_view out, int N, int H,
                                      int W, int C, void* amax_block, void* stream) {
    CVK_CHECK_ARG(amax_block, "cvk_bn_relu_apply_amax: null amax_block");
    return bn_relu_apply_launch("cvk_bn_relu_apply_amax", y, ldy, scale, shift, out, N, H, W, C, amax_block, stream);
}
static int bn_relu_apply_launch(const char* who, const float* y, int ldy, const float* scale, const float* shift, cvk_view out, int N, int H,
                                int W, int C, void* amax, void* stream) {
    CVK_CHECK_ARG(y && scale && shift && out.ptr, "%s: null pointer", who);
    CVK_CHECK_ARG(N > 0 && H > 0 && W > 0 && C > 0 && ldy >= C && (long)N * H * W < (1L << 31), "%s: bad shape", who);
    const int M = N * H * W;
    const PixMap om = make_map(out, H, W);
    const bool v4 = vec_ok(y, out.ptr, scale, ldy, 0, C, &om) && cvk_aligned16(shift);
    const long total = (long)M * (v4 ? C / 4 : C);
    const int cap = amax ? 2048 : 16384;
    const int blocks = (int)((total + 255) / 256 < cap ? (total + 255) / 256 : cap);
    if (v4)
        hipLaunchKernelGGL(k_bn_relu_apply<4>, dim3(blocks), dim3(256), 0, (hipStream_t)stream, y, ldy, scale, shift, out.ptr, om, M, C, (unsigned*)amax);
    else
        hipLaunchKernelGGL(k_bn_relu_apply<1>, dim3(blocks), dim3(256), 0, (hipStream_t)stream, y, ldy, scale, shift, out.ptr, om, M, C, (unsigned*)amax);
    CVK_LAUNCH_RETURN(who);
}

static int bn_relu_apply_pool_launch(const char* who, const float* y, int ldy, const float* scale, const float* shift, cvk_view out, float* pool,
                                     unsigned char* code, int N, int H, int W, int C, void* amax_out, void* amax_pool, void* stream);
extern "C" int cvk_bn_relu_apply_pool(const float* y, int ldy, const float* scale, const float* shift, cvk_view out, float* pool,
                                      unsigned char* code, int N, int H, int W, int C, void* stream) {
    return bn_relu_apply_pool_launch("cvk_bn_relu_apply_pool", y, ldy, scale, shift, out, pool, code, N, H, W, C, nullptr, nullptr, stream);
}
extern "C" int cvk_bn_relu_apply_pool_amax(const float* y, int ldy, const float* scale, const float* shift, cvk_view out, float* pool,
                                           unsigned char* code, int N, int H, int W, int C, void* amax_out, void* amax_pool, void* stream) {
    return bn_relu_apply_pool_launch("cvk_bn_relu_apply_pool_amax", y, ldy, scale, shift, out, pool, code, N, H, W, C, amax_out, amax_pool, stream);
}
static int bn_relu_apply_pool_launch(const char* who, const float* y, int ldy, const float* scale, const float* shift, cvk_view out, float* pool,
                                     unsigned char* code, int N, int H, int W, int C, void* amax_out, void* amax_pool, void* stream) {
    CVK_CHECK_ARG(y && scale && shift && out.ptr && pool, "%s: null pointer", who);
    CVK_CHECK_ARG(N > 0 && H >= 2 && W >= 2 && C > 0 && ldy >= C && (long)N * H * W < (1L << 31), "%s: bad shape", who);
    const PixMap om = make_map(out, H, W);
    const bool v4 = vec_ok(y, out.ptr, scale, ldy, 0, C, &om) && cvk_aligned16(shift) && cvk_aligned16(pool);
    CVK_CHECK_ARG(v4, "%s: needs the 4-channel vector layout", who);
    const long total = (long)N * ((H + 1) / 2) * ((W + 1) / 2) * (C / 4);
    const int cap = (amax_out || amax_pool) ? 2048 : 16384;
    const int blocks = (int)((total + 255) / 256 < cap ? (total + 255) / 256 : cap);
    hipLaunchKernelGGL(k_bn_relu_apply_pool, dim3(blocks), dim3(256), 0, (hipStream_t)stream, y, ldy, scale, shift, out.ptr, om, pool, code, N, H, W, C,
                       (unsigned*)amax_out, (unsigned*)amax_pool);
    CVK_LAUNCH_RETURN(who);
}

extern "C" int cvk_bn_bwd_blocks(int M) {
    if (M <= 0) return 0;
    int pb = cvk_cdiv(M, 16);
    pb = pb < 512 ? pb : 512;
    const int rows = cvk_cdiv(M, pb);
    return cvk_cdiv(M, rows);
}

static int bn_bwd_launch(int mode, cvk_view dout, const float* y, int ldy, const float* scale, const float* shift,
                         const float* mean, const float* rstd, const float* dgamma, const float* dbeta, float* dy, int ld_dy,
                         float* part, int N, int H, int W, int C, int use_batch_stats, void* stream, const char* name, void* amax = nullptr) {
    CVK_CHECK_ARG(dout.ptr && y && scale && shift && mean && rstd, "%s: null pointer", name);
    CVK_CHECK_ARG(N > 0 && H > 0 && W > 0 && C > 0 && ldy >= C && (long)N * H * W < (1L << 31), "%s: bad shape", name);
    const int M = N * H * W;
    const PixMap dm = make_map(dout, H, W);
    bool v4 = vec_ok(y, dout.ptr, scale, ldy, mode == 1 ? ld_dy : 0, C, &dm) && cvk_aligned16(shift) && cvk_aligned16(mean) && cvk_aligned16(rstd);
    if (mode == 1) v4 = v4 && cvk_aligned16(dy);
    const int PB = cvk_bn_bwd_blocks(M), rows = bwd_rows(M);
    const int nb = cvk_cdiv(M, rows);
    const int cchunk = v4 ? 1024 : 256;
    dim3 grid(nb, cvk_cdiv(C, cchunk));
    hipStream_t s = (hipStream_t)stream;
#define CVK_BWD(V_, MODE_)                                                                                              \
    hipLaunchKernelGGL((k_bn_bwd<V_, MODE_>), grid, dim3(256), 0, s, dout.ptr, dm, y, ldy, scale, shift, mean, rstd, dgamma, \
                       dbeta, dy, ld_dy, part, M, C, rows, PB, cchunk, use_batch_stats, (unsigned*)amax)
    if (mode == 0) { if (v4) CVK_BWD(4, 0); else CVK_BWD(1, 0); }
    else { if (v4) CVK_BWD(4, 1); else CVK_BWD(1, 1); }
#undef CVK_BWD
    CVK_LAUNCH_RETURN(name);
}

extern "C" int cvk_bn_bwd_reduce(cvk_view dout, const float* y, int ldy, const float* scale, const float* shift,
                                 const float* mean, const float* rstd, float* part, int N, int H, int W, int C, void* stream) {
    CVK_CHECK_ARG(part, "cvk_bn_bwd_reduce: null partial buffer");
    return bn_bwd_launch(0, dout, y, ldy, scale, shift, mean, rstd, nullptr, nullptr, nullptr, 0, part, N, H, W, C, 1, stream,
                         "cvk_bn_bwd_reduce");
}

extern "C" int cvk_bn_bwd_dx(cvk_view dout, const float* y, int ldy, const float* scale, const float* shift, const float* mean,
                             const float* rstd, const float* dgamma, const float* dbeta, float* dy, int ld_dy, float* dbias_part,
                             int N, int H, int W, int C, int use_batch_stats, void* stream) {
    CVK_CHECK_ARG(dy && ld_dy >= C, "cvk_bn_bwd_dx: bad dy");
    CVK_CHECK_ARG(!use_batch_stats || (dgamma && dbeta), "cvk_bn_bwd_dx: dgamma/dbeta required in training mode");
    return bn_bwd_launch(1, dout, y, ldy, scale, shift, mean, rstd, dgamma, dbeta, dy, ld_dy, dbias_part, N, H, W, C,
                         use_batch_stats, stream, "cvk_bn_bwd_dx");
}

extern "C" int cvk_bn_bwd_dx_amax(cvk_view dout, const float* y, int ldy, const float* scale, const float* shift, const float* mean,
                                  const float* rstd, const float* dgamma, const float* dbeta, float* dy, int ld_dy, float* dbias_part,
                                  int N, int H, int W, int C, int use_batch_stats, void* amax_block, void* stream) {
    CVK_CHECK_ARG(dy && ld_dy >= C && amax_block, "cvk_bn_bwd_dx_amax: bad dy / amax_block");
    CVK_CHECK_ARG(!use_batch_stats || (dgamma && dbeta), "cvk_bn_bwd_dx_amax: dgamma/dbeta required in training mode");
    return bn_bwd_launch(1, dout, y, ldy, scale, shift, mean, rstd, dgamma, dbeta, dy, ld_dy, dbias_part, N, H, W, C,
                         use_batch_stats, stream, "cvk_bn_bwd_dx_amax", amax_block);
}

extern "C" int cvk_bn_bwd_e_blocks(int N, int H, int W) {
    if (N <= 0 || H <= 0 || W <= 0) return 0;
    const int Mt = N * H * ((W + 3) / 4);
    const int pb = cvk_bn_bwd_blocks(N * H * W);
    const int tiles = cvk_cdiv(Mt, pb);
    return cvk_cdiv(Mt, tiles);
}

static int bn_bwd_dx_e_launch(const char* who, int six, cvk_view dout, const float* y, int ldy, const float* scale, const float* shift, const float* mean,
                              const float* rstd, const float* dgamma, const float* dbeta, float* dy, int ld_dy, float* E,
                              float* part, int N, int H, int W, int C, int use_batch_stats, void* amax, void* stream);
extern "C" int cvk_bn_bwd_dx_e(cvk_view dout, const float* y, int ldy, const float* scale, const float* shift, const float* mean,
                               const float* rstd, const float* dgamma, const float* dbeta, float* dy, int ld_dy, float* E,
                               float* part, int N, int H, int W, int C, int use_batch_stats, void* stream) {
    return bn_bwd_dx_e_launch("cvk_bn_bwd_dx_e", 0, dout, y, ldy, scale, shift, mean, rstd, dgamma, dbeta, dy, ld_dy, E, part, N, H, W, C, use_batch_stats,
                              nullptr, stream);
}
extern "C" int cvk_bn_bwd_dx_e_amax(int six, cvk_view dout, const float* y, int ldy, const float* scale, const float* shift, const float* mean,
                                    const float* rstd, const float* dgamma, const float* dbeta, float* dy, int ld_dy, float* E,
                                    float* part, int N, int H, int W, int C, int use_batch_stats, void* amax_block, void* stream) {
    CVK_CHECK_ARG(amax_block, "cvk_bn_bwd_dx_e_amax: null amax block");
    return bn_bwd_dx_e_launch("cvk_bn_bwd_dx_e_amax", six == 2 ? 2 : (six ? 1 : 0), dout, y, ldy, scale, shift, mean, rstd, dgamma, dbeta, dy, ld_dy, E, part, N, H, W, C,
                              use_batch_stats, amax_block, stream);
}
static int bn_bwd_dx_e_launch(const char* who, int six, cvk_view dout, const float* y, int ldy, const float* scale, const float* shift, const float* mean,
                              const float* rstd, const float* dgamma, const float* dbeta, float* dy, int ld_dy, float* E,
                              float* part, int N, int H, int W, int C, int use_batch_stats, void* amax, void* stream) {
    if (six) {
        CVK_CHECK_ARG(dout.ptr && y && scale && shift && mean && rstd && dy && E && dgamma && dbeta, "%s: null pointer", who);
        CVK_CHECK_ARG(N > 0 && H > 0 && W > 0 && C > 0 && ldy >= C && ld_dy == C && (long)N * H * W < (1L << 31), "%s: bad shape (ld_dy must equal C)", who);
        const PixMap dm6 = make_map(dout, H, W);
        const bool v46 = vec_ok(y, dout.ptr, scale, ldy, ld_dy, C, &dm6) && cvk_aligned16(shift) && cvk_aligned16(mean) &&
                         cvk_aligned16(rstd) && cvk_aligned16(dy) && cvk_aligned16(E);
        CVK_CHECK_ARG(v46, "%s: needs the 4-channel vector layout (use cvk_bn_bwd_dx)", who);
        const int M6 = N * H * W, Wt6 = (W + 3) / 4, Mt6 = N * H * Wt6;
        const int Wtp = (Wt6 + 7) / 8 * 8;
        const long rows = (long)N * (H + 2) * Wtp + 2L * Wtp;
        const int pb6 = cvk_bn_bwd_blocks(M6);
        const int tiles6 = cvk_cdiv(Mt6, pb6), nb6 = cvk_cdiv(Mt6, tiles6);
        dim3 grid6(nb6, cvk_cdiv(C, 1024));
        hipLaunchKernelGGL(k_bn_bwd_dx_e, grid6, dim3(256), 0, (hipStream_t)stream, dout.ptr, dm6, y, ldy, scale, shift, mean, rstd,
                           dgamma, dbeta, dy, ld_dy, E, part, M6, C, W, Wt6, Mt6, tiles6, 1024, use_batch_stats, H, Wtp, six == 2 ? -rows : rows, (unsigned*)amax);
        CVK_LAUNCH_RETURN(who);
    }
    CVK_CHECK_ARG(dout.ptr && y && scale && shift && mean && rstd && dy && E && dgamma && dbeta, "%s: null pointer", who);
    CVK_CHECK_ARG(N > 0 && H > 0 && W > 0 && C > 0 && ldy >= C && ld_dy >= C && (long)N * H * W < (1L << 31), "%s: bad shape", who);
    const PixMap dm = make_map(dout, H, W);
    const bool v4 = vec_ok(y, dout.ptr, scale, ldy, ld_dy, C, &dm) && cvk_aligned16(shift) && cvk_aligned16(mean) &&
                    cvk_aligned16(rstd) && cvk_aligned16(dy) && cvk_aligned16(E);
    CVK_CHECK_ARG(v4, "%s: needs the 4-channel vector layout (use cvk_bn_bwd_dx)", who);
    const int M = N * H * W, Wt = (W + 3) / 4, Mt = N * H * Wt;
    const int pb = cvk_bn_bwd_blocks(M);
    const int tiles = cvk_cdiv(Mt, pb), nb = cvk_cdiv(Mt, tiles);
    const int cchunk = 1024;
    dim3 grid(nb, cvk_cdiv(C, cchunk));
    hipLaunchKernelGGL(k_bn_bwd_dx_e, grid, dim3(256), 0, (hipStream_t)stream, dout.ptr, dm, y, ldy, scale, shift, mean, rstd,
                       dgamma, dbeta, dy, ld_dy, E, part, M, C, W, Wt, Mt, tiles, cchunk, use_batch_stats, 0, 0, 0L, (unsigned*)amax);
    CVK_LAUNCH_RETURN(who);
}

extern "C" int cvk_bn_bwd_dx_e6(cvk_view dout, const float* y, int ldy, const float* scale, const float* shift, const float* mean,
                                const float* rstd, const float* dgamma, const float* dbeta, float* dy, int ld_dy, float* E6,
                                float* part, int N, int H, int W, int C, int use_batch_stats, void* stream) {
    return bn_bwd_dx_e_launch("cvk_bn_bwd_dx_e6", 1, dout, y, ldy, scale, shift, mean, rstd, dgamma, dbeta, dy, ld_dy, E6, part, N, H, W, C, use_batch_stats,
                              nullptr, stream);
}

extern "C" int cvk_bn_bwd_dx_e4p(cvk_view dout, const float* y, int ldy, const float* scale, const float* shift, const float* mean,
                                 const float* rstd, const float* dgamma, const float* dbeta, float* dy, int ld_dy, float* E4p,
                                 float* part, int N, int H, int W, int C, int use_batch_stats, void* stream) {
    return bn_bwd_dx_e_launch("cvk_bn_bwd_dx_e4p", 2, dout, y, ldy, scale, shift, mean, rstd, dgamma, dbeta, dy, ld_dy, E4p, part, N, H, W, C, use_batch_stats,
                              nullptr, stream);
}

extern "C" int cvk_colsum_finalize_batch(const cvk_colsum_job* jobs, int n, void* stream) {
    CVK_CHECK_ARG(jobs && n > 0 && n <= CVK_COLSUM_BATCH_MAX, "cvk_colsum_finalize_batch: 1 <= n <= %d jobs", CVK_COLSUM_BATCH_MAX);
    ColsumJobsDev d;
    int cmax = 0;
    for (int i = 0; i < n; ++i) {
        CVK_CHECK_ARG(jobs[i].part && jobs[i].out && jobs[i].PB > 0 && jobs[i].C > 0, "cvk_colsum_finalize_batch: bad job %d", i);
        d.j[i] = jobs[i];
        if (jobs[i].C > cmax) cmax = jobs[i].C;
    }
    hipLaunchKernelGGL(k_colsum_finalize_batch, dim3(cvk_cdiv(cmax, 64), n), dim3(1024), 0, (hipStream_t)stream, d);
    CVK_LAUNCH_RETURN("cvk_colsum_finalize_batch");
}

extern "C" int cvk_colsum_finalize(const float* part, int PB, int C, float* out0, float* out1, void* stream) {
    CVK_CHECK_ARG(part && out0 && PB > 0 && C > 0, "cvk_colsum_finalize: bad arguments");
    hipLaunchKernelGGL(k_colsum_finalize, dim3(cvk_cdiv(C, 64), out1 ? 2 : 1), dim3(1024), 0, (hipStream_t)stream, part, PB, C, out0, out1);
    CVK_LAUNCH_RETURN("cvk_colsum_finalize");
}
```

### pytorch-camvid_amd/csrc/wgradp.hip

```cpp
#include "conv_tile.h"
#include "lds_dma.h"
#include <utility>

namespace {

template <int... Ks, class F>
__device__ __forceinline__ void p_static_for(std::integer_sequence<int, Ks...>, F&& f) {
    (f(std::integral_constant<int, Ks>{}), ...);
}

__device__ __forceinline__ void p_dma16(const void* sbase, unsigned voff, unsigned lds_byte_addr) {
    asm volatile("s_mov_b32 m0, %2\n\ts_nop 0\n\tglobal_load_lds_dwordx4 %0, %1" : : "v"(voff), "s"(sbase), "s"(lds_byte_addr) : "memory");
}

__host__ __device__ inline long p_rows(int N, int H, int Wtp) { return (long)N * (H + 2) * Wtp + 2L * Wtp; }

template <int MODE, bool SM = false>
__global__ __launch_bounds__(256) void k_wgradp_planes(const float* __restrict__ X, int ld, float* __restrict__ P, int N, int H, int W,
                                                      int Wt, int Wtp, int C) {
    const int cvn = C >> 2;
    const long rows = p_rows(N, H, Wtp);
    const long idx = (long)blockIdx.x * 256 + threadIdx.x;
    if (idx >= rows * cvn) return;
    const long row = idx / cvn;
    const int c = (int)(idx - row * cvn) * 4;
    const f32x4 z = {0.f, 0.f, 0.f, 0.f};
    f32x4 v[6] = {z, z, z, z, z, z};
    const long q = row - Wtp;
    if (q >= 0 && q < (long)N * (H + 2) * Wtp) {
        const int xt = (int)(q % Wtp);
        const long ry = q / Wtp;
        const int yp = (int)(ry % (H + 2)), n = (int)(ry / (H + 2));
        if (yp >= 1 && yp <= H && xt < Wt) {
            const float* p = X + (((size_t)n * H + (yp - 1)) * W + 4 * (size_t)xt) * ld + c;
            if (MODE == 0) {
                f32x4 d[6];
#pragma unroll
                for (int j = 0; j < 6; ++j) {
                    const int col = 4 * xt - 1 + j;
                    d[j] = (col >= 0 && col < W) ? *reinterpret_cast<const f32x4*>(p + (long)(j - 1) * ld) : z;
                }
                const f32x4 a = d[4] - 4.f * d[2], b = d[3] - 4.f * d[1], e = d[4] - d[2], f = d[3] - d[1];
                v[0] = 4.f * d[0] - 5.f * d[2] + d[4];
                v[1] = a + b;
                v[2] = a - b;
                v[3] = e + 2.f * f;
                v[4] = e - 2.f * f;
                v[5] = 4.f * d[1] - 5.f * d[3] + d[5];
            } else {
                f32x4 d[4];
#pragma unroll
                for (int i = 0; i < 4; ++i) d[i] = (4 * xt + i < W) ? *reinterpret_cast<const f32x4*>(p + (long)i * ld) : z;
                const f32x4 a = d[0] + d[2], b = d[1] + d[3], cc = d[0] + 4.f * d[2], dd = 2.f * d[1] + 8.f * d[3];
                v[0] = d[0];
                v[1] = a + b;
                v[2] = a - b;
                v[3] = cc + dd;
                v[4] = cc - dd;
                v[5] = d[3];
            }
        }
    }
    float* o = SM ? P + ((size_t)(c >> 4) * rows + (size_t)row) * 16 + (c & 15) : P + (size_t)row * C + c;
    const size_t ps = (size_t)rows * C;
#pragma unroll
    for (int x = 0; x < 6; ++x) *reinterpret_cast<f32x4*>(o + x * ps) = v[x];
}

template <bool SM = false>
__global__ __launch_bounds__(256) void k_wgradp_zero_pads(float* __restrict__ P, int N, int H, int Wt, int Wtp, int C, int nplanes) {
    const int cvn = C >> 2;
    const long rows = p_rows(N, H, Wtp);
    const int padc = Wtp - Wt;
    const long n_end = 2L * Wtp, n_border = (long)N * 2 * Wtp, n_col = (long)N * H * padc;
    const long idx = (long)blockIdx.x * 256 + threadIdx.x;
    const long pr = idx / cvn;
    const int c = (int)(idx - pr * cvn) * 4;
    if (pr >= n_end + n_border + n_col) return;
    long row;
    if (pr < n_end) {
        row = pr < Wtp ? pr : rows - Wtp + (pr - Wtp);
    } else if (pr < n_end + n_border) {
        const long k = pr - n_end;
        const int n = (int)(k / (2 * Wtp)), rem = (int)(k - (long)n * 2 * Wtp);
        const int yp = rem < Wtp ? 0 : H + 1, xt = rem < Wtp ? rem : rem - Wtp;
        row = (long)Wtp + ((long)n * (H + 2) + yp) * Wtp + xt;
    } else {
        const long k = pr - n_end - n_border;
        const long ry = k / padc;
        const int xt = Wt + (int)(k - ry * padc);
        const int n = (int)(ry / H), yy = (int)(ry - (long)n * H);
        row = (long)Wtp + ((long)n * (H + 2) + yy + 1) * Wtp + xt;
    }
    const f32x4 z = {0.f, 0.f, 0.f, 0.f};
    const size_t ps = (size_t)rows * C;
    for (int x = 0; x < nplanes; ++x)
        *reinterpret_cast<f32x4*>(P + x * ps + (SM ? ((size_t)(c >> 4) * rows + (size_t)row) * 16 + (c & 15) : (size_t)row * C + c)) = z;
}

template <bool VSM, bool EDY>
__global__ __launch_bounds__(64, 2) void k_wgradp_gemm(const float* __restrict__ E6, const float* __restrict__ V6, float* __restrict__ slab,
                                                      int H, int Wtp, int Cin_ld, int Cout, long rows, int Q, int runs, int nci, int nco,
                                                      const float* __restrict__ dy, int W, int njobs) {
    __shared__ __attribute__((aligned(1024))) char smem[12 * 1024];
    const unsigned smem_addr = cvk_lds_addr(smem);
    const int lane = threadIdx.x;
    const int lj = lane & 15, kq = lane >> 4;

    const int per = 6 * nci * nco;
    for (int job = blockIdx.x; job < njobs; job += gridDim.x) {
        asm volatile("s_waitcnt vmcnt(0) lgkmcnt(0)" ::: "memory");
        const int id = cvk_xcd_remap(job, njobs);
        const int run = id / per, u = id - run * per;
        const int xi = u % 6, cit = (u / 6) % nci, cot = u / (6 * nci);
        const int qb = (int)((long)run * Q / runs), qe = (int)((long)(run + 1) * Q / runs);
        if (qb >= qe) continue;
        const int so = Wtp >> 3;

        const bool edy = EDY && (xi == 0 || xi == 5);
        const float* const Eb = edy ? dy + cot * 64 + (xi == 5 ? 3 * Cout : 0) : E6 + (size_t)(EDY ? xi - 1 : xi) * rows * Cout + cot * 64;
        const int epitch = edy ? 4 * Cout : Cout;
        const float* const Vb = V6 + (size_t)xi * rows * Cin_ld + (VSM ? (size_t)cit * 4 * rows * 16 : (size_t)cit * 64);
        const int vpitch = VSM ? 16 : Cin_ld;
        const unsigned evoff = (unsigned)(((lane >> 4) * epitch + (lane & 15) * 4) * 4);
        const unsigned vvoff = VSM ? (unsigned)((((unsigned long)((lane & 15) >> 2) * (unsigned long)rows + (lane >> 4)) * 16 + (lane & 3) * 4) * 4)
                                   : (unsigned)(((lane >> 4) * Cin_ld + (lane & 15) * 4) * 4);
        auto block_row = [&](int strip, int yp) -> long {
            const int n = strip / so, xg = strip - n * so;
            return (long)Wtp + ((long)n * (H + 2) + yp) * Wtp + 8 * xg;
        };
        auto dma_V = [&](int strip, int yp) {
            const float* src = Vb + (size_t)block_row(strip, yp) * vpitch;
            const unsigned dst = smem_addr + (yp & 3) * 2048;
            p_dma16(src, vvoff, dst);
            p_dma16(src + 4 * (size_t)vpitch, vvoff, dst + 1024);
        };
        auto dma_E = [&](int strip, int yp, int slot) {
            const int en = strip / so, exg = strip - en * so;
            const float* src = edy ? Eb + (((size_t)en * H + (yp - 1)) * W + 32 * (size_t)exg) * Cout : Eb + (size_t)block_row(strip, yp) * Cout;
            const unsigned dst = smem_addr + 8192 + slot * 2048;
            p_dma16(src, evoff, dst);
            p_dma16(src + 4 * (size_t)epitch, evoff, dst + 1024);
        };

        f32x4 acc[3][16];
#pragma unroll
        for (int r = 0; r < 3; ++r)
#pragma unroll
            for (int b = 0; b < 16; ++b) acc[r][b] = f32x4{0.f, 0.f, 0.f, 0.f};

        const int frag = kq * 256 + lj * 16;

        int strip = qb / H, y = qb - strip * H;
        dma_V(strip, y);
        dma_V(strip, y + 1);
        dma_V(strip, y + 2);
        dma_E(strip, y + 1, 0);
        int es = 0;
        for (int q = qb; q < qe; ++q) {
            const bool last_in_strip = (y == H - 1);
            const bool more = q + 1 < qe;
            asm volatile("s_waitcnt lgkmcnt(0)" ::: "memory");
            if (more && !last_in_strip) {
                dma_V(strip, y + 3);
                dma_E(strip, y + 2, es ^ 1);
                cvk_wait_vm<4>();
            } else {
                cvk_wait_vm<0>();
            }
            __builtin_amdgcn_s_setprio(1);
            const char* const eblk = smem + 8192 + es * 2048;
            const char* const v0 = smem + ((y + 0) & 3) * 2048;
            const char* const v1 = smem + ((y + 1) & 3) * 2048;
            const char* const v2 = smem + ((y + 2) & 3) * 2048;
#pragma unroll
            for (int ks = 0; ks < 2; ++ks) {
// ... 255 lines not shown
```

### pytorch-camvid_amd/engine.py

```python
import ctypes
import os
from collections import namedtuple

import torch

from . import _lib
from ._lib import View, ViewH, check
from .route import conv_route, pad4, split_fmt
from .route import layer_tile, wgrad2d_pays, wino2d_ok, wino2d_pays, wino4_pays

_F32, _BF16 = torch.float32, torch.bfloat16


class ActBuf:
    __slots__ = ("id", "N", "H", "W", "C", "ld", "name", "dtype")

    def __init__(self, id_, N, H, W, C, name="", dtype=_F32):
        self.id, self.N, self.H, self.W, self.C, self.name, self.dtype = id_, N, H, W, C, name, dtype
        self.ld = pad4(C) if dtype == _F32 else max(32, (C + 7) // 8 * 8)

    @property
    def esize(self):
        return 4 if self.dtype == _F32 else 2

# ... 420 lines not shown
        self._reads(src_buf)
        op = self.add(Unpool(src_buf, pool_op, dst))
        op.wants = self._needs_grad(src_buf)
        self._writes(dst, 0, dst.C, op)
        return dst

    def upsample(self, src_buf):
        dst = self.new_buf(src_buf.C, 2 * src_buf.H, 2 * src_buf.W, "up")
        self._reads(src_buf)
        op = self.add(Upsample(src_buf, dst))
        op.wants = self._needs_grad(src_buf)
        self._writes(dst, 0, dst.C, op)
        return dst

    def zero_frame(self, view):
        self.add(ZeroFrame(view))

    def seal(self, thin=True):
        if self.bf16:
            b = self.output.buf
            if not self.output.is_full:
                raise NotImplementedError("bf16 mode: the network output must be a whole buffer")
            b.dtype = _F32
            b.ld = pad4(b.C)
            readers = [op for op in self.ops if getattr(op, "src", None) is self.input]
            if (thin and not self.input_needs_grad and self.input.C <= 4 and readers and self.input is not self.output.buf
                    and all(isinstance(op, ConvBnRelu) and op.cout == 64 for op in readers)
                    and self.input.H * self.input.W * 64 * 2 < 2 ** 31):
                self.input.ld = 8


_SPLIT_ENV_LOGGED = False


def _split_mode_from_env():
    global _SPLIT_ENV_LOGGED
    raw = os.environ.get("CVK_W2D_SPLIT")
    if raw is None:
        return 0
    modes = {"0": 0, "1": 3, "3": 3, "2": 2}
    if raw.strip() not in modes:
        raise ValueError(f"CVK_W2D_SPLIT={raw!r}: allowed values are 0 (off, the default), 2 (two fp16 terms) and 3 or 1 (three bf16 terms); "
                         "or leave it unset and call pytorch_camvid_amd.set_split_operands(net, mode)")
    mode = modes[raw.strip()]
    if mode and not _SPLIT_ENV_LOGGED:
        _SPLIT_ENV_LOGGED = True
        import sys
        print(f"pytorch_camvid_amd: CVK_W2D_SPLIT={raw} — fp32 convolution products run as split {'fp16 x 2' if mode == 2 else 'bf16 x 3'} operands "
              "(opt-in, not the exact-fp32 default)", file=sys.stderr)
    return mode


class Runner:

    def __init__(self):
        self.lib = _lib.load()
        self._ws = None
        self._dp_wgs = None
        self._collectives_in_flight = False
        self.grad_sync = None
        self.accumulator = None
        self.wino = WINO_DEFAULT
        self.wino4 = WINO4_DEFAULT
        self.wino4f = WINO4F_DEFAULT
        self.wgradp = WGRADP_DEFAULT
        self.vplanes = VPLANES_DEFAULT
        self.thin = os.environ.get("CVK_THIN", "1") != "0"
        self.pool_bnred = os.environ.get("CVK_POOL_BNRED", "1") != "0"
        self.wino2d = WINO2D_DEFAULT
        self.w2d_split = _split_mode_from_env()
        self.w2tile_cfg = W2TILE_DEFAULT
        self.w2tile = 6
        self.w2tile_dgrad = 6
        self.bf16 = False
        self.wcache = WCACHE_DEFAULT
        self.wepoch = 0
        self._wc = {}
        self._wjobs, self._wjobs_cfg = {}, None
        self._pass_token = 0
        self._passes = 0
        self.wcache_builds = 0
        self.wgrad_side = os.environ.get("CVK_WGRAD_SIDE", WGRAD_SIDE_DEFAULT) != "0"
        self.side_families = WGRAD_SIDE_FAMILIES

    def side_allowed(self, fold):
        return (self.wgrad_side and not self.bf16 and self.grad_sync is None and self.accumulator is None and fold is None and PROF is None
                and not torch.cuda.is_current_stream_capturing())

    def side_begin(self, st, *keep):
        s = self.lib.cvk_side_begin(st.stream)
        if not s:
            check(-1, "cvk_side_begin")
        st.side_keep.extend(k for k in keep if k is not None)
        st.side_open = True
        return s

    def side_join(self, st):
        if st.side_open:
            check(self.lib.cvk_side_join(st.stream), "cvk_side_join")
            st.side_open = False
            st.side_keep.clear()

    def persistent_wgs(self):
        gs = self.grad_sync
        if gs is None or (getattr(gs, "world", 1) <= 1 and not getattr(gs, "always_issue", False)):
            return 0
        if self._dp_wgs is None:
            cus = torch.cuda.get_device_properties(torch.cuda.current_device()).multi_processor_count
            self._dp_wgs = max(8, cus - int(os.environ.get("CVK_DP_RESERVE_CUS", "8")))
        return self._dp_wgs

    def launch_wgs(self):
        return self.persistent_wgs() if self._collectives_in_flight else 0

    def derived(self, key, src, build, job=None):
        if not self.wcache or key is None or torch.cuda.is_current_stream_capturing():
            self.wcache_builds += 1
            return build()
        if job is not None:
            self._wjobs[key] = (src, job)
        return self._cache(key, src, build)

    def _cache(self, key, src, build=None):
        sig = (WEIGHT_EPOCH[0], self.wepoch, src.data_ptr(), src._version, self._pass_token)
        ent = self._wc.get(key)
        if (ent is None or ent[0] != sig) and build is not None:
            ent = self._wc[key] = (sig, build())
            self.wcache_builds += 1
        return ent[1] if ent is not None and ent[0] == sig else None

    def prebuild_fp32(self, plan, st, need_grad):
        if not self.wcache or torch.cuda.is_current_stream_capturing():
            return
        cfg = (id(plan),) + self.kernel_config()
        if cfg != self._wjobs_cfg:
            self._wjobs, self._wjobs_cfg = {}, cfg
            return
        live = {p.data_ptr() for p in st.params}
        lib, fam_jobs = self.lib, {"w4f": [], "w2d": []}
        for key, (src, (fam, floats, rows, cols, tile, dgrad)) in self._wjobs.items():
            if src.data_ptr() not in live or (dgrad and not need_grad):
                continue
            if self._cache(key, src) is not None:
                continue
            t = self._cache(key, src, lambda: _empty(floats, src.device))
            fam_jobs[fam].append((_lib.WtJob(src.data_ptr(), t.data_ptr(), rows, cols, tile, dgrad), 4.0 * (src.numel() + floats)))
        for fam, fn in (("w4f", lib.cvk_wino4f_weight_transform_batch), ("w2d", lib.cvk_w2d_weight_transform_batch)):
            jobs = fam_jobs[fam]
            for i in range(0, len(jobs), _lib.WT_BATCH_MAX):
                chunk = jobs[i:i + _lib.WT_BATCH_MAX]
                arr = (_lib.WtJob * len(chunk))(*[j for j, _ in chunk])
                _timed(self, "k_weight_transform_batch", sum(b for _, b in chunk),
                       lambda: check(fn(ctypes.addressof(arr), len(chunk), st.stream), "cvk_%s_weight_transform_batch" % fam), "byte")

    def prepack_bf16(self, plan, st, need_grad):
        if not self.wcache or torch.cuda.is_current_stream_capturing():
            return
        lib, jobs, keep = self.lib, [], []
        for op in plan.ops:
            if not isinstance(op, ConvBnRelu):
                continue
            w = st.params[4 * op.pslot]
            for key, dgrad, rows, kpad in op.packs_wanted(self, need_grad):
                if self._cache(key, w) is not None:
                    continue
                wc = channels_last(w)
# ... 37 lines not shown
            return
        arr = (_lib.WReduceJob * len(st.wreduces))(*[_lib.WReduceJob(sl.data_ptr(), dw, n, sp, 0) for sl, sp, n, dw in st.wreduces])
        check(self.lib.cvk_wgrad_reduce_bf16s_batch(ctypes.addressof(arr), len(st.wreduces), st.stream), "cvk_wgrad_reduce_bf16s_batch")
        st.wreduces.clear()

    def flush_colsums(self, st):
        if not st.colsums:
            return
        arr = (_lib.ColsumJob * len(st.colsums))(*[_lib.ColsumJob(p.data_ptr(), o, pb, c) for p, pb, c, o in st.colsums])
        check(self.lib.cvk_colsum_finalize_batch(ctypes.addressof(arr), len(st.colsums), st.stream), "cvk_colsum_finalize_batch")
        st.colsums.clear()

    def grads_ready(self, st, slot):
        if st.sync is not None and st.plan.convs[slot].trainable:
            if st.sync.closes_bucket():
                self.flush_colsums(st)
                self.flush_wreduces(st)
            st.sync.layer_done(st, slot)
            self._collectives_in_flight = st.sync.in_flight()

    def begin_sync(self, st, plan, fold=None):
        gs = self.grad_sync
        if gs is None:
            return None
        if not gs.enabled or (fold is not None and not fold.closing):
            gs.launched = []
            return None
        return gs.begin(st, plan)

    def import_nchw(self, st, x, buf, dtype, zero_pad=False):
        xp = x.permute(0, 2, 3, 1)
        if dtype == _F32 and buf.ld == buf.C and xp.is_contiguous():
            return xp
        t = (torch.zeros if zero_pad and buf.ld != buf.C else torch.empty)((buf.N, buf.H, buf.W, buf.ld), device=x.device, dtype=dtype)
        fn = "cvk_import_nchw_bf16" if dtype == _BF16 else "cvk_import_nchw"
        check(getattr(self.lib, fn)(x.data_ptr(), *x.stride(), t.data_ptr(), buf.ld, buf.N, buf.C, buf.H, buf.W, st.stream), fn)
        return t

    def plan_amax(self, plan, st):
        if split_fmt(self) != 2 or plan.bf16 or not (st.training and st.need_grad):
            return
        routes = self.routes(plan, True, True)
        layers = [op for op in plan.ops if isinstance(op, ConvBnRelu) and (routes[op.idx].split or (op.src.ld % 32 == 0 and op.cout % 4 == 0))]
        if not layers:
            return

        def writers(buf):
            out = []
            for op in plan.ops:
                if isinstance(op, ConvBnRelu) and (op.dst.buf is buf or (op.pool_dst is buf and op.cout % 4 == 0)):
                    out.append(op)
                elif isinstance(op, (MaxPool, Unpool, Upsample)) and op.dst is buf and not (isinstance(op, MaxPool) and op.fused):
                    out.append(op)
                elif isinstance(op, ZeroFrame) and op.view.buf is buf:
                    out.append(op)
            return out

        want, ok = [], {}

        def fusable(buf):
            if buf.id in ok:
                return ok[buf.id]
            ok[buf.id] = False
            ws = writers(buf)
            good = bool(ws) and buf is not plan.input
            for op in ws:
                if isinstance(op, Upsample):
                    good = good and fusable(op.src)
                elif not isinstance(op, (ConvBnRelu, ZeroFrame)):
                    good = False
            ok[buf.id] = good
            if good:
                want.append(buf)
            return good
        for op in layers:
            fusable(op.src)
        blocks = amax_blocks(self.lib, len(want) + len(layers), st.device)
        for i, buf in enumerate(want):
            st.amax[buf.id] = blocks[i]
        st.amax_spare = blocks[len(want):]

    def kernel_config(self):
        return (self.wino, self.wino4, self.wino4f, self.wino2d, self.wgradp, self.vplanes, self.thin, self.pool_bnred, self.w2d_split,
                self.w2tile_cfg)

    def routes(self, plan, training, need_grad):
        key = (self.kernel_config(), training, need_grad)
        r = plan.routes.get(key)
        if r is None:
            if split_fmt(self):
                check_bn_modes(plan, training, "set_split_operands")
            self.w2tile, self.w2tile_dgrad = self.tile_for(plan)
            r = plan.routes[key] = {op.idx: conv_route(self, op, training, need_grad) for op in plan.ops if isinstance(op, ConvBnRelu)}
        return r

    def tile_for(self, plan):
        if self.w2tile_cfg in (4, 6):
            return self.w2tile_cfg, self.w2tile_cfg
        return (4, 6) if any(isinstance(op, Unpool) for op in plan.ops) else (6, 6)

    def forward(self, plan, x, params, training, need_grad):
        dev = x.device
        self._collectives_in_flight = False
        st = RunState(params, training, need_grad)
        st.device = dev
        st.plan = plan
        if training and need_grad:
            self._passes += 1
            st.pass_token = self._passes
        self._pass_token = st.pass_token
        st.stream = torch.cuda.current_stream(dev).cuda_stream
        st.act[plan.input.id] = self.import_nchw(st, x, plan.input, _BF16 if plan.bf16 else _F32)
        if plan.bf16:
            check_bn_modes(plan, training, "bf16 mode", need_grad, forward_only_ok=True)
            self.prepack_bf16(plan, st, need_grad)
        else:
            st.routes = self.routes(plan, training, need_grad)
            self.prebuild_fp32(plan, st, need_grad)
            self.plan_amax(plan, st)
        for op in plan.ops:
            _CUR_OP[0] = (op.idx, "fwd")
            op.fwd(self, st)
        _CUR_OP[0] = None
        ov = plan.output
        out = st.act[ov.buf.id][..., :ov.buf.C].permute(0, 3, 1, 2)
        if not need_grad:
            st.act.clear()
            st.saved.clear()
        return out, st

    def backward(self, plan, st, gout):
        dev = gout.device
        st.stream = torch.cuda.current_stream(dev).cuda_stream
        self._pass_token = st.pass_token
        params = st.params
        st.goffs, total = layout_grads(params)
        st.gflat = torch.empty(total, device=dev, dtype=_F32)
        fold = st.fold = self.accumulator.open_pass(st, plan, total) if self.accumulator is not None else None
        st.sync = self.begin_sync(st, plan, fold)
        self._collectives_in_flight = False
        st.side = self.side_allowed(fold)
        st.grad[plan.output.buf.id] = self.import_nchw(st, gout, plan.output.buf, _F32, zero_pad=True)
        try:
            for op in reversed(plan.ops):
                _CUR_OP[0] = (op.idx, "bwd")
                op.bwd(self, st)
        finally:
            _CUR_OP[0] = None
            self.side_join(st)
        self.flush_colsums(st)
        self.flush_wreduces(st)
        if fold is not None and st.sync is None:
            fold.whole(st)
        dx = None
        if plan.input_needs_grad:
            gi = st.grad[plan.input.id]
            dx = gi[..., :plan.input.C].permute(0, 3, 1, 2)
            if plan.bf16:
                dx = dx.float()
        grads = []
        hand_out = fold is None or fold.closing
        for i, p in enumerate(params):
            op = plan.convs[i // 4]
            if not hand_out or not (op.w_req, op.b_req, op.g_req, op.be_req)[i % 4]:
                grads.append(None)
                continue
            n = p.numel()
# ... 68 lines not shown
```

Before: 251.7 images/s.

## Fuse pad zeroing and BN-backward column-sum finalize into the BN dx kernels

Adds BN-backward dx/E kernel variants that zero the wgradp pad rows themselves (the Z path) instead of issuing separate zero launches. It also adds variants that reduce the partial sums for dgamma/dbeta inside each block (the FIN path) instead of running a separate colsum_finalize kernel. The default CVK_BWD_CHAIN=z enables only the pad-zero fusion; FIN is opt-in. The aim is fewer kernel launches per BN layer in backward, at the cost of extra per-block work (every block repeats the FIN reduction) and more complex host-side fallbacks.

After: 252.0 images/s (median of 4 runs). Within noise of the previous version (+0.1%).

```diff
diff --git a/include/cvk.h b/include/cvk.h
--- a/include/cvk.h
+++ b/include/cvk.h
@@ -228,6 +228,22 @@
 int cvk_bn_bwd_dx(cvk_view dout, const float* y, int ldy, const float* scale, const float* shift,
                   const float* mean, const float* rstd, const float* dgamma, const float* dbeta,
                   float* dy, int ld_dy, float* dbias_part, int N, int H, int W, int C, int use_batch_stats, void* stream);
+int cvk_bn_bwd_dx_e6_z(cvk_view dout, const float* y, int ldy, const float* scale, const float* shift, const float* mean,
+                       const float* rstd, const float* dgamma, const float* dbeta, float* dy, int ld_dy, float* E6, float* part,
+                       int N, int H, int W, int C, int use_batch_stats, void* stream);
+int cvk_bn_bwd_dx_e4p_z(cvk_view dout, const float* y, int ldy, const float* scale, const float* shift, const float* mean,
+                        const float* rstd, const float* dgamma, const float* dbeta, float* dy, int ld_dy, float* E4p, float* part,
+                        int N, int H, int W, int C, int use_batch_stats, void* stream);
+int cvk_bn_bwd_dx_e_z_amax(int six, cvk_view dout, const float* y, int ldy, const float* scale, const float* shift, const float* mean,
+                           const float* rstd, const float* dgamma, const float* dbeta, float* dy, int ld_dy, float* E, float* part, int N, int H,
+                           int W, int C, int use_batch_stats, void* amax_block, void* stream);
+int cvk_bn_bwd_fin_supported(int C);
+int cvk_bn_bwd_dx_fin(cvk_view dout, const float* y, int ldy, const float* scale, const float* shift, const float* mean,
+                      const float* rstd, const float* sums, int PBs, float* dgamma, float* dbeta, float* dy, int ld_dy,
+                      float* dbias_part, int N, int H, int W, int C, int use_batch_stats, void* amax_block, void* stream);
+int cvk_bn_bwd_dx_e_fin(int mode, cvk_view dout, const float* y, int ldy, const float* scale, const float* shift, const float* mean,
+                        const float* rstd, const float* sums, int PBs, float* dgamma, float* dbeta, float* dy, int ld_dy, float* E,
+                        float* part, int N, int H, int W, int C, int use_batch_stats, void* amax_block, void* stream);
 
 int cvk_maxpool2x2_fwd(cvk_view x, float* out, uint8_t* code, int N, int H, int W, int C, void* stream);
 int cvk_maxpool2x2_bwd(const float* dout, cvk_view x, const uint8_t* code, cvk_view dx, int accumulate,
diff --git a/pytorch-camvid_amd/_lib.py b/pytorch-camvid_amd/_lib.py
--- a/pytorch-camvid_amd/_lib.py
+++ b/pytorch-camvid_amd/_lib.py
@@ -168,6 +168,17 @@
                                      c_int, c_int, c_int, c_int, c_int, c_vp, c_vp]),
     "cvk_bn_bwd_dx_amax": (c_int, [View, c_vp, c_int, c_vp, c_vp, c_vp, c_vp, c_vp, c_vp, c_vp, c_int, c_vp,
                                    c_int, c_int, c_int, c_int, c_int, c_vp, c_vp]),
+    "cvk_bn_bwd_dx_e6_z": (c_int, [View, c_vp, c_int, c_vp, c_vp, c_vp, c_vp, c_vp, c_vp, c_vp, c_int, c_vp, c_vp,
+                                   c_int, c_int, c_int, c_int, c_int, c_vp]),
+    "cvk_bn_bwd_dx_e4p_z": (c_int, [View, c_vp, c_int, c_vp, c_vp, c_vp, c_vp, c_vp, c_vp, c_vp, c_int, c_vp, c_vp,
+                                    c_int, c_int, c_int, c_int, c_int, c_vp]),
+    "cvk_bn_bwd_dx_e_z_amax": (c_int, [c_int, View, c_vp, c_int, c_vp, c_vp, c_vp, c_vp, c_vp, c_vp, c_vp, c_int, c_vp, c_vp,
+                                       c_int, c_int, c_int, c_int, c_int, c_vp, c_vp]),
+    "cvk_bn_bwd_fin_supported": (c_int, [c_int]),
+    "cvk_bn_bwd_dx_fin": (c_int, [View, c_vp, c_int, c_vp, c_vp, c_vp, c_vp, c_vp, c_int, c_vp, c_vp, c_vp, c_int, c_vp,
+                                  c_int, c_int, c_int, c_int, c_int, c_vp, c_vp]),
+    "cvk_bn_bwd_dx_e_fin": (c_int, [c_int, View, c_vp, c_int, c_vp, c_vp, c_vp, c_vp, c_vp, c_int, c_vp, c_vp, c_vp, c_int, c_vp, c_vp,
+                                    c_int, c_int, c_int, c_int, c_int, c_vp, c_vp]),
     "cvk_maxpool2x2_fwd": (c_int, [View, c_vp, c_vp, c_int, c_int, c_int, c_int, c_vp]),
     "cvk_maxpool2x2_bwd": (c_int, [c_vp, View, c_vp, View, c_int, c_int, c_int, c_int, c_int, c_vp]),
     "cvk_maxpool2x2_bwd_bnred_blocks": (c_int, [c_int, c_int, c_int, c_int]),
diff --git a/pytorch-camvid_amd/conv_bf16.py b/pytorch-camvid_amd/conv_bf16.py
--- a/pytorch-camvid_amd/conv_bf16.py
+++ b/pytorch-camvid_amd/conv_bf16.py
@@ -20,6 +20,7 @@
 class ConvBnReluBf16(ConvBnRelu):
     _pitch, _ydt = staticmethod(int), _BF16
     _BN = ("cvk_bn_bwd_blocks_bf16", "cvk_bn_bwd_reduce_bf16", "k_bnbwd_bf16<reduce>")
+    _FIN = False
 
     def thin_mode(self, R, dgrad, ld_dy=0):
         if not R.thin or self.src.H * self.src.W * max(self.src.ld, self.cout, ld_dy, 64) * 2 >= 2 ** 31:
@@ -94,7 +95,7 @@
     def _dout(self, st):
         return self.dst.hview(st.grad[self.dst.buf.id]), 1 if self.dst.buf.dtype == _F32 else 0
 
-    def _bn_bwd(self, R, st, rt, bn, gg, gbe, part, PB, gb):
+    def _bn_bwd(self, R, st, rt, bn, gg, gbe, part, PB, fin, gb):
         src, C, ld_dy = self.src, self.cout, max(32, self.cout)
         dy = torch.empty(src.M * ld_dy, device=st.device, dtype=_BF16)
         _timed(R, "k_bnbwd_bf16<dx>", ((4.0 if bn[1] else 2.0) + 4.0) * src.M * C, lambda: check(
diff --git a/pytorch-camvid_amd/conv_fp32.py b/pytorch-camvid_amd/conv_fp32.py
--- a/pytorch-camvid_amd/conv_fp32.py
+++ b/pytorch-camvid_amd/conv_fp32.py
@@ -325,6 +325,7 @@
 class ConvBnRelu(Op):
     _pitch, _ydt = staticmethod(pad4), _F32
     _BN = ("cvk_bn_bwd_blocks", "cvk_bn_bwd_reduce", "k_bn_bwd<reduce>")
+    _FIN = True
 
     def __init__(self, src, dst, pslot, holder, cin, cout, src_needs_grad, bn_train=True, req=(True, True, True, True)):
         self.src, self.dst, self.pslot, self.holder = src, dst, pslot, holder
@@ -456,49 +457,91 @@
     def _bn_sums(self, R, st, bn, gg, gbe):
         lib, s, src, C, (blocks, fn, name) = R.lib, st.stream, self.src, self.cout, self._BN
         PB = getattr(lib, blocks)(src.M)
-        part = _empty(2 * PB * C, st.device)
+        need_dy = self.w_req or self.b_req or self.src_needs_grad
+        fin = (self._FIN and R.chain_fin and need_dy and self.bn_train and pad4(C) == C and bool(lib.cvk_bn_bwd_fin_supported(C)))
+        part = _empty((3 if fin else 2) * PB * C, st.device)
+        dpart = part[2 * PB * C:] if fin else part
         pre = st.bnred.pop(self.idx, None)
         if pre is not None:
+            if fin:
+                return dpart, PB, pre
             check(lib.cvk_colsum_finalize(pre[0].data_ptr(), pre[1], C, gbe, gg, s), "cvk_colsum_finalize")
         elif self.bn_train or self.g_req or self.be_req:
             _timed(R, name, float(self.dst.buf.esize + self._ydt.itemsize) * src.M * C, lambda: check(
                 getattr(lib, fn)(*bn, part.data_ptr(), src.N, src.H, src.W, C, s), fn), "byte")
+            if fin:
+                return dpart, PB, (part, PB)
             check(lib.cvk_colsum_finalize(part.data_ptr(), PB, C, gbe, gg, s), "cvk_colsum_finalize")
-        if self.w_req or self.b_req or self.src_needs_grad:
-            return part, PB
+        if need_dy:
+            return part, PB, None
         R.grads_ready(st, self.pslot)
         return None
 
     _BN_E = {"dx+E": (0, "cvk_bn_bwd_dx_e", 16.0), "dx+E6": (1, "cvk_bn_bwd_dx_e6", 24.0), "dx+E4p": (2, "cvk_bn_bwd_dx_e4p", 16.0)}
 
-    def _bn_bwd(self, R, st, rt, bn, gg, gbe, part, PB, gb):
+    def _bn_bwd(self, R, st, rt, bn, gg, gbe, part, PB, fin, gb):
         lib, s, src, kind = R.lib, st.stream, self.src, rt.bn_bwd
         N, H, W, M, C, ldy = src.N, src.H, src.W, src.M, self.cout, pad4(self.cout)
+        ubs = 1 if self.bn_train else 0
         if kind == "dx+E4p":
             dyb = _empty(M * ldy + lib.cvk_wgradp_dy_slack(W) * ldy, st.device)
-            dyb[M * ldy:].zero_()
             dy = dyb[:M * ldy]
         else:
             dy = torch.zeros(M * ldy, device=st.device, dtype=_F32) if ldy != C else _empty(M * ldy, st.device)
         want_amax = rt.dy_amax and bool(st.amax_spare)
-        head, tail = (*bn, gg, gbe, dy.data_ptr(), ldy), (part.data_ptr(), N, H, W, C, 1 if self.bn_train else 0)
+        head, tail = (*bn, gg, gbe, dy.data_ptr(), ldy), (part.data_ptr(), N, H, W, C, ubs)
+        fhead = (*bn, fin[0].data_ptr(), fin[1], gg, gbe, dy.data_ptr(), ldy) if fin is not None else None
+
+        def unfin():
+            nonlocal fin
+            check(lib.cvk_colsum_finalize(fin[0].data_ptr(), fin[1], C, gbe, gg, s), "cvk_colsum_finalize")
+            fin = None
         if kind != "dx":
             mode, plain, eb = self._BN_E[kind]
-            if kind == "dx+E":
+            padded = kind != "dx+E"
+            if padded:
+                prows = lib.cvk_wgradp_plane_rows(N, H, W)
+                E = _empty((4 if mode == 2 else 6) * prows * C, st.device)
+                zbytes = 4.0 * ((4 if mode == 2 else 6) * (prows - N * H * ((W + 3) // 4)) + (lib.cvk_wgradp_dy_slack(W) if mode == 2 else 0)) * C
+            else:
                 E = _empty(4 * N * H * ((W + 3) // 4) * ldy, st.device)
-            else:
-                E = _empty((4 if mode == 2 else 6) * lib.cvk_wgradp_plane_rows(N, H, W) * C, st.device)
+            blk = st.amax_spare[-1] if want_amax else None
+            bp = blk.data_ptr() if blk is not None else None
+            nbytes = (12.0 * M + eb * N * H * ((W + 3) // 4)) * C
+            z = padded and R.chain_z
+
+            def zero_launches():
+                if kind == "dx+E4p":
+                    dyb[M * ldy:].zero_()
                 check((lib.cvk_wgradp_zero_pads4 if mode == 2 else lib.cvk_wgradp_zero_pads)(E.data_ptr(), N, H, W, C, s), "cvk_wgradp_zero_pads")
-            blk = st.amax_spare[-1] if want_amax else None
-            rc = _timed(R, "k_bn_bwd<%s>" % kind, (12.0 * M + eb * N * H * ((W + 3) // 4)) * C, lambda: (
-                lib.cvk_bn_bwd_dx_e_amax(mode, *head, E.data_ptr(), *tail, blk.data_ptr(), s) if blk is not None
-                else getattr(lib, plain)(*head, E.data_ptr(), *tail, s)), "byte")
+            rc = -1
+            if z or fin is not None:
+                if padded and not z:
+                    zero_launches()
+                rc = _timed(R, "k_bn_bwd<%s>" % kind, nbytes + (zbytes if z else 0.0), lambda: (
+                    lib.cvk_bn_bwd_dx_e_fin(mode + (2 if z else 0), *fhead, E.data_ptr(), *tail, bp, s) if fin is not None
+                    else lib.cvk_bn_bwd_dx_e_z_amax(mode, *head, E.data_ptr(), *tail, bp, s) if blk is not None
+                    else getattr(lib, plain + "_z")(*head, E.data_ptr(), *tail, s)), "byte")
+                if rc != 0 and fin is not None:
+                    unfin()
+            if rc != 0:
+                if padded:
+                    zero_launches()
+                rc = _timed(R, "k_bn_bwd<%s>" % kind, nbytes, lambda: (
+                    lib.cvk_bn_bwd_dx_e_amax(mode, *head, E.data_ptr(), *tail, bp, s) if blk is not None
+                    else getattr(lib, plain)(*head, E.data_ptr(), *tail, s)), "byte")
             if rc == 0:
                 if gb is not None:
                     R.defer_colsum(st, part, lib.cvk_bn_bwd_e_blocks(N, H, W), C, gb)
                 return dy, E, (st.amax_spare.pop() if blk is not None else None)
         am = st.amax_spare.pop() if want_amax else None
-        _timed(R, "k_bn_bwd<dx>", 12.0 * M * C, lambda: check(amax_call(lib, "cvk_bn_bwd_dx", (*head, *tail), (am,), s), "cvk_bn_bwd_dx"), "byte")
+        if fin is not None:
+            rc = _timed(R, "k_bn_bwd<dx>", 12.0 * M * C, lambda: lib.cvk_bn_bwd_dx_fin(
+                *fhead, *tail, am.data_ptr() if am is not None else None, s), "byte")
+            if rc != 0:
+                unfin()
+        if fin is None:
+            _timed(R, "k_bn_bwd<dx>", 12.0 * M * C, lambda: check(amax_call(lib, "cvk_bn_bwd_dx", (*head, *tail), (am,), s), "cvk_bn_bwd_dx"), "byte")
         if gb is not None:
             R.defer_colsum(st, part, PB, C, gb)
         return dy, None, am
diff --git a/pytorch-camvid_amd/csrc/bn.hip b/pytorch-camvid_amd/csrc/bn.hip
--- a/pytorch-camvid_amd/csrc/bn.hip
+++ b/pytorch-camvid_amd/csrc/bn.hip
@@ -1,4 +1,5 @@
 #include "cvk_common.h"
+#include "wgradp_pads.h"
 
 namespace {
 
@@ -232,17 +233,97 @@
     if (amax_pool != nullptr) { __syncthreads(); cvk_amax_publish_wg(mxp, amax_pool, snapp); }
 }
 
-template <int V, int MODE>
+#define CVK_FIN_CMAX 128
+struct BnFin {
+    const float* sums;
+    int PB;
+    float* out_dbeta;
+    float* out_dgamma;
+};
+struct BnFinLds {
+    double red[2 * 16 * CVK_FIN_CMAX];
+    float fin[2][CVK_FIN_CMAX];
+};
+
+#define FIN_NI 4
+__device__ __forceinline__ void bn_fin_sums(const BnFin& F, int C, BnFinLds& L, bool store) {
+    const int t = threadIdx.x, PB = F.PB;
+    const int per = (32 * C) >> 8;
+    const unsigned C16 = 16u * C;
+    for (int k0 = 0; k0 < per; k0 += FIN_NI) {
+        double a[FIN_NI][4];
+        unsigned off[FIN_NI];
+        int g[FIN_NI];
+#pragma unroll
+        for (int i = 0; i < FIN_NI; ++i) {
+            const int idx = t + 256 * (k0 + i), wg = idx / C, c = idx - wg * C;
+            g[i] = wg & 15;
+            off[i] = (unsigned)(((wg >> 4) * PB + g[i]) * C + c);
+            a[i][0] = a[i][1] = a[i][2] = a[i][3] = 0.0;
+        }
+        int q = 0;
+        for (; q + 63 < PB; q += 64) {
+            const float* sq = F.sums + (size_t)q * C;
+            float v[FIN_NI][4];
+#pragma unroll
+            for (int i = 0; i < FIN_NI; ++i)
+#pragma unroll
+                for (int k = 0; k < 4; ++k) v[i][k] = sq[off[i] + k * C16];
+#pragma unroll
+            for (int i = 0; i < FIN_NI; ++i)
+#pragma unroll
+                for (int k = 0; k < 4; ++k) a[i][k] += (double)v[i][k];
+        }
+#pragma unroll
+        for (int i = 0; i < FIN_NI; ++i) {
+            const float* si = F.sums + (off[i] - (unsigned)(g[i] * C));
+            int p = q + g[i];
+            for (; p + 48 < PB; p += 64) {
+                a[i][0] += (double)si[(size_t)p * C];
+                a[i][1] += (double)si[(size_t)(p + 16) * C];
+                a[i][2] += (double)si[(size_t)(p + 32) * C];
+                a[i][3] += (double)si[(size_t)(p + 48) * C];
+            }
+            for (; p < PB; p += 16) a[i][0] += (double)si[(size_t)p * C];
+            L.red[t + 256 * (k0 + i)] = (a[i][0] + a[i][1]) + (a[i][2] + a[i][3]);
+        }
+    }
+    __syncthreads();
+    for (int j = t; j < 2 * C; j += 256) {
+        const int which = j / C, c = j - which * C;
+        double s = 0.0;
+#pragma unroll
+        for (int i = 0; i < 16; ++i) s += L.red[(which * 16 + i) * C + c];
+        const float f = (float)s;
+        L.fin[which][c] = f;
+        if (store) (which == 0 ? F.out_dbeta : F.out_dgamma)[c] = f;
+    }
+    __syncthreads();
+}
+
+template <bool FIN>
+__device__ __forceinline__ BnFinLds* bn_fin_lds() {
+    if constexpr (FIN) {
+        __shared__ BnFinLds L;
+        return &L;
+    } else {
+        return nullptr;
+    }
+}
+
+template <int V, int MODE, bool FIN = false>
 __global__ __launch_bounds__(256) void k_bn_bwd(const float* __restrict__ dout, PixMap dm, const float* __restrict__ y, int ldy,
                                                const float* __restrict__ scale, const float* __restrict__ shift,
                                                const float* __restrict__ mean, const float* __restrict__ rstd,
                                                const float* __restrict__ dgamma, const float* __restrict__ dbeta,
                                                float* __restrict__ dy, int ld_dy, float* __restrict__ part, int M, int C,
-                                               int rows, int PB, int cchunk, int use_batch_stats, unsigned* __restrict__ amax) {
+                                               int rows, int PB, int cchunk, int use_batch_stats, unsigned* __restrict__ amax, BnFin fin) {
     typedef typename Vec<V>::T VT;
     __shared__ float red[2][256 * V];
     float mx = 0.f;
     const unsigned snap = MODE == 1 ? cvk_amax_snapshot(amax) : 0u;
+    BnFinLds* const fl = bn_fin_lds<FIN>();
+    if (FIN && use_batch_stats) bn_fin_sums(fin, C, *fl, blockIdx.x == 0);
     const int c0 = blockIdx.y * cchunk;
     const int cw = min(cchunk, C - c0);
     const int cvn = cw / V;
@@ -266,8 +347,8 @@
             const float invM = 1.f / (float)M;
 #pragma unroll
             for (int j = 0; j < V; ++j) {
-                k1[j] = use_batch_stats ? dbeta[c + j] * invM : 0.f;
-                k2[j] = use_batch_stats ? dgamma[c + j] * invM : 0.f;
+                k1[j] = use_batch_stats ? (FIN ? fl->fin[0][c + j] : dbeta[c + j]) * invM : 0.f;
+                k2[j] = use_batch_stats ? (FIN ? fl->fin[1][c + j] : dgamma[c + j]) * invM : 0.f;
             }
         }
 #pragma unroll 4
@@ -315,6 +396,7 @@
     }
 }
 
+template <bool Z = false, bool FIN = false>
 __global__ __launch_bounds__(256) void k_bn_bwd_dx_e(const float* __restrict__ dout, PixMap dm, const float* __restrict__ y, int ldy,
                                                     const float* __restrict__ scale, const float* __restrict__ shift,
                                                     const float* __restrict__ mean, const float* __restrict__ rstd,
@@ -322,10 +404,31 @@
                                                     float* __restrict__ dy, int ld_dy, float* __restrict__ E,
                                                     float* __restrict__ part, int M, int C, int W, int Wt, int Mt, int tiles,
                                                     int cchunk, int use_batch_stats, int six_H, int six_Wtp, long six_rows,
-                                                    unsigned* __restrict__ amax) {
+                                                    unsigned* __restrict__ amax, int nb, int slackv, BnFin fin) {
+    if (Z && (int)blockIdx.x >= nb) {
+        if (blockIdx.y != 0) return;
+        const int cvnz = C >> 2, N = Mt / (six_H * Wt);
+        const long prows = six_rows < 0 ? -six_rows : six_rows;
+        const int np = six_rows < 0 ? 4 : 6;
+        const long total = cvk_wgradp_pad_count(N, six_H, Wt, six_Wtp) * cvnz;
+        const f32x4 z = {0.f, 0.f, 0.f, 0.f};
+        for (long idx = (long)(blockIdx.x - nb) * 256 + threadIdx.x; idx < total + slackv; idx += (long)(gridDim.x - nb) * 256) {
+            if (idx < total) {
+                const long pr = idx / cvnz;
+                const int cz = (int)(idx - pr * cvnz) * 4;
+                float* o = E + (size_t)cvk_wgradp_pad_row(pr, N, six_H, Wt, six_Wtp) * C + cz;
+                for (int x = 0; x < np; ++x) *reinterpret_cast<f32x4*>(o + (size_t)x * prows * C) = z;
+            } else {
+                *reinterpret_cast<f32x4*>(dy + (size_t)M * ld_dy + (size_t)(idx - total) * 4) = z;
+            }
+        }
+        return;
+    }
     __shared__ float red[256 * 4];
     float mx = 0.f;
     const unsigned snap = cvk_amax_snapshot(amax);
+    BnFinLds* const fl = bn_fin_lds<FIN>();
+    if (FIN && use_batch_stats) bn_fin_sums(fin, C, *fl, blockIdx.x == 0);
     const int c0 = blockIdx.y * cchunk;
     const int cw = min(cchunk, C - c0);
     const int cvn = cw / 4;
@@ -345,7 +448,10 @@
         if (use_batch_stats) {
             const float invM = 1.f / (float)M;
 #pragma unroll
-            for (int j = 0; j < 4; ++j) { k1[j] = dbeta[c + j] * invM; k2[j] = dgamma[c + j] * invM; }
+            for (int j = 0; j < 4; ++j) {
+                k1[j] = (FIN ? fl->fin[0][c + j] : dbeta[c + j]) * invM;
+                k2[j] = (FIN ? fl->fin[1][c + j] : dgamma[c + j]) * invM;
+            }
         }
         const size_t plane = (size_t)Mt * ld_dy;
         for (int tl = tbeg + pr; tl < tend; tl += ppp) {
@@ -610,7 +716,8 @@
 
 static int bn_bwd_launch(int mode, cvk_view dout, const float* y, int ldy, const float* scale, const float* shift,
                          const float* mean, const float* rstd, const float* dgamma, const float* dbeta, float* dy, int ld_dy,
-                         float* part, int N, int H, int W, int C, int use_batch_stats, void* stream, const char* name, void* amax = nullptr) {
+                         float* part, int N, int H, int W, int C, int use_batch_stats, void* stream, const char* name, void* amax = nullptr,
+                         const BnFin* fin = nullptr) {
     CVK_CHECK_ARG(dout.ptr && y && scale && shift && mean && rstd, "%s: null pointer", name);
     CVK_CHECK_ARG(N > 0 && H > 0 && W > 0 && C > 0 && ldy >= C && (long)N * H * W < (1L << 31), "%s: bad shape", name);
     const int M = N * H * W;
@@ -624,8 +731,13 @@
     hipStream_t s = (hipStream_t)stream;
 #define CVK_BWD(V_, MODE_)                                                                                              \
     hipLaunchKernelGGL((k_bn_bwd<V_, MODE_>), grid, dim3(256), 0, s, dout.ptr, dm, y, ldy, scale, shift, mean, rstd, dgamma, \
-                       dbeta, dy, ld_dy, part, M, C, rows, PB, cchunk, use_batch_stats, (unsigned*)amax)
-    if (mode == 0) { if (v4) CVK_BWD(4, 0); else CVK_BWD(1, 0); }
+                       dbeta, dy, ld_dy, part, M, C, rows, PB, cchunk, use_batch_stats, (unsigned*)amax, BnFin{})
+    if (fin != nullptr) {
+        CVK_CHECK_ARG(mode == 1 && v4, "%s: needs the 4-channel vector layout (use cvk_colsum_finalize + cvk_bn_bwd_dx)", name);
+        hipLaunchKernelGGL((k_bn_bwd<4, 1, true>), grid, dim3(256), 0, s, dout.ptr, dm, y, ldy, scale, shift, mean, rstd, nullptr, nullptr, dy, ld_dy,
+                           part, M, C, rows, PB, cchunk, use_batch_stats, (unsigned*)amax, *fin);
+    }
+    else if (mode == 0) { if (v4) CVK_BWD(4, 0); else CVK_BWD(1, 0); }
     else { if (v4) CVK_BWD(4, 1); else CVK_BWD(1, 1); }
 #undef CVK_BWD
     CVK_LAUNCH_RETURN(name);
@@ -666,7 +778,8 @@
 
 static int bn_bwd_dx_e_launch(const char* who, int six, cvk_view dout, const float* y, int ldy, const float* scale, const float* shift, const float* mean,
                               const float* rstd, const float* dgamma, const float* dbeta, float* dy, int ld_dy, float* E,
-                              float* part, int N, int H, int W, int C, int use_batch_stats, void* amax, void* stream);
+                              float* part, int N, int H, int W, int C, int use_batch_stats, void* amax, void* stream, bool z = false,
+                              const BnFin* fin = nullptr);
 extern "C" int cvk_bn_bwd_dx_e(cvk_view dout, const float* y, int ldy, const float* scale, const float* shift, const float* mean,
                                const float* rstd, const float* dgamma, const float* dbeta, float* dy, int ld_dy, float* E,
                                float* part, int N, int H, int W, int C, int use_batch_stats, void* stream) {
@@ -682,7 +795,10 @@
 }
 static int bn_bwd_dx_e_launch(const char* who, int six, cvk_view dout, const float* y, int ldy, const float* scale, const float* shift, const float* mean,
                               const float* rstd, const float* dgamma, const float* dbeta, float* dy, int ld_dy, float* E,
-                              float* part, int N, int H, int W, int C, int use_batch_stats, void* amax, void* stream) {
+                              float* part, int N, int H, int W, int C, int use_batch_stats, void* amax, void* stream, bool z, const BnFin* fin) {
+    CVK_CHECK_ARG(!z || six, "%s: only the padded-plane passes zero their pads", who);
+    if (fin != nullptr) dgamma = fin->out_dgamma, dbeta = fin->out_dbeta;
+    const BnFin F = fin != nullptr ? *fin : BnFin{};
     if (six) {
         CVK_CHECK_ARG(dout.ptr && y && scale && shift && mean && rstd && dy && E && dgamma && dbeta, "%s: null pointer", who);
         CVK_CHECK_ARG(N > 0 && H > 0 && W > 0 && C > 0 && ldy >= C && ld_dy == C && (long)N * H * W < (1L << 31), "%s: bad shape (ld_dy must equal C)", who);
@@ -695,9 +811,17 @@
         const long rows = (long)N * (H + 2) * Wtp + 2L * Wtp;
         const int pb6 = cvk_bn_bwd_blocks(M6);
         const int tiles6 = cvk_cdiv(Mt6, pb6), nb6 = cvk_cdiv(Mt6, tiles6);
-        dim3 grid6(nb6, cvk_cdiv(C, 1024));
-        hipLaunchKernelGGL(k_bn_bwd_dx_e, grid6, dim3(256), 0, (hipStream_t)stream, dout.ptr, dm6, y, ldy, scale, shift, mean, rstd,
-                           dgamma, dbeta, dy, ld_dy, E, part, M6, C, W, Wt6, Mt6, tiles6, 1024, use_batch_stats, H, Wtp, six == 2 ? -rows : rows, (unsigned*)amax);
+        const int slackv = z && six == 2 ? (4 * Wtp - W + 4) * (C / 4) : 0;
+        const long zthreads = z ? cvk_wgradp_pad_count(N, H, Wt6, Wtp) * (C / 4) + slackv : 0;
+        const int nz = (int)((zthreads + 255) / 256 < 256 ? (zthreads + 255) / 256 : 256);
+        dim3 grid6(nb6 + nz, cvk_cdiv(C, 1024));
+#define CVK_BWD_E6(Z_, FIN_)                                                                                                                 \
+    hipLaunchKernelGGL((k_bn_bwd_dx_e<Z_, FIN_>), grid6, dim3(256), 0, (hipStream_t)stream, dout.ptr, dm6, y, ldy, scale, shift, mean, rstd, \
+                       dgamma, dbeta, dy, ld_dy, E, part, M6, C, W, Wt6, Mt6, tiles6, 1024, use_batch_stats, H, Wtp, six == 2 ? -rows : rows, \
+                       (unsigned*)amax, nb6, slackv, F)
+        if (z) { if (fin) CVK_BWD_E6(true, true); else CVK_BWD_E6(true, false); }
+        else { if (fin) CVK_BWD_E6(false, true); else CVK_BWD_E6(false, false); }
+#undef CVK_BWD_E6
         CVK_LAUNCH_RETURN(who);
     }
     CVK_CHECK_ARG(dout.ptr && y && scale && shift && mean && rstd && dy && E && dgamma && dbeta, "%s: null pointer", who);
@@ -711,8 +835,12 @@
     const int tiles = cvk_cdiv(Mt, pb), nb = cvk_cdiv(Mt, tiles);
     const int cchunk = 1024;
     dim3 grid(nb, cvk_cdiv(C, cchunk));
-    hipLaunchKernelGGL(k_bn_bwd_dx_e, grid, dim3(256), 0, (hipStream_t)stream, dout.ptr, dm, y, ldy, scale, shift, mean, rstd,
-                       dgamma, dbeta, dy, ld_dy, E, part, M, C, W, Wt, Mt, tiles, cchunk, use_batch_stats, 0, 0, 0L, (unsigned*)amax);
+    if (fin)
+        hipLaunchKernelGGL((k_bn_bwd_dx_e<false, true>), grid, dim3(256), 0, (hipStream_t)stream, dout.ptr, dm, y, ldy, scale, shift, mean, rstd,
+                           dgamma, dbeta, dy, ld_dy, E, part, M, C, W, Wt, Mt, tiles, cchunk, use_batch_stats, 0, 0, 0L, (unsigned*)amax, nb, 0, F);
+    else
+        hipLaunchKernelGGL((k_bn_bwd_dx_e<false, false>), grid, dim3(256), 0, (hipStream_t)stream, dout.ptr, dm, y, ldy, scale, shift, mean, rstd,
+                           dgamma, dbeta, dy, ld_dy, E, part, M, C, W, Wt, Mt, tiles, cchunk, use_batch_stats, 0, 0, 0L, (unsigned*)amax, nb, 0, F);
     CVK_LAUNCH_RETURN(who);
 }
 
@@ -728,6 +856,60 @@
                                  float* part, int N, int H, int W, int C, int use_batch_stats, void* stream) {
     return bn_bwd_dx_e_launch("cvk_bn_bwd_dx_e4p", 2, dout, y, ldy, scale, shift, mean, rstd, dgamma, dbeta, dy, ld_dy, E4p, part, N, H, W, C, use_batch_stats,
                               nullptr, stream);
+}
+
+extern "C" int cvk_bn_bwd_dx_e6_z(cvk_view dout, const float* y, int ldy, const float* scale, const float* shift, const float* mean,
+                                  const float* rstd, const float* dgamma, const float* dbeta, float* dy, int ld_dy, float* E6,
+                                  float* part, int N, int H, int W, int C, int use_batch_stats, void* stream) {
+    return bn_bwd_dx_e_launch("cvk_bn_bwd_dx_e6_z", 1, dout, y, ldy, scale, shift, mean, rstd, dgamma, dbeta, dy, ld_dy, E6, part, N, H, W, C, use_batch_stats,
+                              nullptr, stream, true);
+}
+extern "C" int cvk_bn_bwd_dx_e4p_z(cvk_view dout, const float* y, int ldy, const float* scale, const float* shift, const float* mean,
+                                   const float* rstd, const float* dgamma, const float* dbeta, float* dy, int ld_dy, float* E4p,
+                                   float* part, int N, int H, int W, int C, int use_batch_stats, void* stream) {
+    return bn_bwd_dx_e_launch("cvk_bn_bwd_dx_e4p_z", 2, dout, y, ldy, scale, shift, mean, rstd, dgamma, dbeta, dy, ld_dy, E4p, part, N, H, W, C,
+                              use_batch_stats, nullptr, stream, true);
+}
+extern "C" int cvk_bn_bwd_dx_e_z_amax(int six, cvk_view dout, const float* y, int ldy, const float* scale, const float* shift, const float* mean,
+                                      const float* rstd, const float* dgamma, const float* dbeta, float* dy, int ld_dy, float* E,
+                                      float* part, int N, int H, int W, int C, int use_batch_stats, void* amax_block, void* stream) {
+    CVK_CHECK_ARG(amax_block && (six == 1 || six == 2), "cvk_bn_bwd_dx_e_z_amax: null amax block or six not 1 / 2");
+    return bn_bwd_dx_e_launch("cvk_bn_bwd_dx_e_z_amax", six, dout, y, ldy, scale, shift, mean, rstd, dgamma, dbeta, dy, ld_dy, E, part, N, H, W, C,
+                              use_batch_stats, amax_block, stream, true);
+}
+
+extern "C" int cvk_bn_bwd_fin_supported(int C) { return C > 0 && C % 64 == 0 && C <= CVK_FIN_CMAX; }
+static int bn_fin_check(const char* who, BnFin* F, const float* sums, int PBs, float* dgamma, float* dbeta, const float* part, long part_rows, int C,
+                        int use_batch_stats) {
+    CVK_CHECK_ARG(cvk_bn_bwd_fin_supported(C), "%s: C %% 64 == 0 and C <= %d (use cvk_colsum_finalize and the plain pass)", who, CVK_FIN_CMAX);
+    CVK_CHECK_ARG(dgamma && dbeta, "%s: null dgamma / dbeta", who);
+    CVK_CHECK_ARG(!use_batch_stats || (sums && PBs > 0), "%s: partial sums required in training mode", who);
+    if (use_batch_stats && part != nullptr) {
+        const float* se = sums + (size_t)2 * PBs * C;
+        CVK_CHECK_ARG(part + (size_t)part_rows * C <= sums || part >= se, "%s: part overlaps the partial sums", who);
+    }
+    *F = BnFin{sums, PBs, dbeta, dgamma};
+    return CVK_OK;
+}
+extern "C" int cvk_bn_bwd_dx_fin(cvk_view dout, const float* y, int ldy, const float* scale, const float* shift, const float* mean,
+                                 const float* rstd, const float* sums, int PBs, float* dgamma, float* dbeta, float* dy, int ld_dy,
+                                 float* dbias_part, int N, int H, int W, int C, int use_batch_stats, void* amax_block, void* stream) {
+    CVK_CHECK_ARG(dy && ld_dy >= C && N > 0 && H > 0 && W > 0 && (long)N * H * W < (1L << 31), "cvk_bn_bwd_dx_fin: bad dy / shape");
+    BnFin F;
+    const int rc = bn_fin_check("cvk_bn_bwd_dx_fin", &F, sums, PBs, dgamma, dbeta, dbias_part, cvk_bn_bwd_blocks(N * H * W), C, use_batch_stats);
+    if (rc != CVK_OK) return rc;
+    return bn_bwd_launch(1, dout, y, ldy, scale, shift, mean, rstd, nullptr, nullptr, dy, ld_dy, dbias_part, N, H, W, C, use_batch_stats, stream,
+                         "cvk_bn_bwd_dx_fin", amax_block, &F);
+}
+extern "C" int cvk_bn_bwd_dx_e_fin(int mode, cvk_view dout, const float* y, int ldy, const float* scale, const float* shift, const float* mean,
+                                   const float* rstd, const float* sums, int PBs, float* dgamma, float* dbeta, float* dy, int ld_dy, float* E,
+                                   float* part, int N, int H, int W, int C, int use_batch_stats, void* amax_block, void* stream) {
+    CVK_CHECK_ARG(mode >= 0 && mode <= 4 && N > 0 && H > 0 && W > 0 && (long)N * H * W < (1L << 31), "cvk_bn_bwd_dx_e_fin: bad mode / shape");
+    BnFin F;
+    const int rc = bn_fin_check("cvk_bn_bwd_dx_e_fin", &F, sums, PBs, dgamma, dbeta, part, cvk_bn_bwd_e_blocks(N, H, W), C, use_batch_stats);
+    if (rc != CVK_OK) return rc;
+    return bn_bwd_dx_e_launch("cvk_bn_bwd_dx_e_fin", mode >= 3 ? mode - 2 : mode, dout, y, ldy, scale, shift, mean, rstd, nullptr, nullptr, dy, ld_dy, E, part,
+                              N, H, W, C, use_batch_stats, amax_block, stream, mode >= 3, &F);
 }
 
 extern "C" int cvk_colsum_finalize_batch(const cvk_colsum_job* jobs, int n, void* stream) {
diff --git a/pytorch-camvid_amd/csrc/wgradp.hip b/pytorch-camvid_amd/csrc/wgradp.hip
--- a/pytorch-camvid_amd/csrc/wgradp.hip
+++ b/pytorch-camvid_amd/csrc/wgradp.hip
@@ -1,5 +1,6 @@
 #include "conv_tile.h"
 #include "lds_dma.h"
+#include "wgradp_pads.h"
 #include <utility>
 
 namespace {
@@ -13,7 +14,7 @@
     asm volatile("s_mov_b32 m0, %2\n\ts_nop 0\n\tglobal_load_lds_dwordx4 %0, %1" : : "v"(voff), "s"(sbase), "s"(lds_byte_addr) : "memory");
 }
 
-__host__ __device__ inline long p_rows(int N, int H, int Wtp) { return (long)N * (H + 2) * Wtp + 2L * Wtp; }
+__host__ __device__ inline long p_rows(int N, int H, int Wtp) { return cvk_wgradp_rows(N, H, Wtp); }
 
 template <int MODE, bool SM = false>
 __global__ __launch_bounds__(256) void k_wgradp_planes(const float* __restrict__ X, int ld, float* __restrict__ P, int N, int H, int W,
@@ -71,27 +72,11 @@
 __global__ __launch_bounds__(256) void k_wgradp_zero_pads(float* __restrict__ P, int N, int H, int Wt, int Wtp, int C, int nplanes) {
     const int cvn = C >> 2;
     const long rows = p_rows(N, H, Wtp);
-    const int padc = Wtp - Wt;
-    const long n_end = 2L * Wtp, n_border = (long)N * 2 * Wtp, n_col = (long)N * H * padc;
     const long idx = (long)blockIdx.x * 256 + threadIdx.x;
     const long pr = idx / cvn;
     const int c = (int)(idx - pr * cvn) * 4;
-    if (pr >= n_end + n_border + n_col) return;
-    long row;
-    if (pr < n_end) {
-        row = pr < Wtp ? pr : rows - Wtp + (pr - Wtp);
-    } else if (pr < n_end + n_border) {
-        const long k = pr - n_end;
-        const int n = (int)(k / (2 * Wtp)), rem = (int)(k - (long)n * 2 * Wtp);
-        const int yp = rem < Wtp ? 0 : H + 1, xt = rem < Wtp ? rem : rem - Wtp;
-        row = (long)Wtp + ((long)n * (H + 2) + yp) * Wtp + xt;
-    } else {
-        const long k = pr - n_end - n_border;
-        const long ry = k / padc;
-        const int xt = Wt + (int)(k - ry * padc);
-        const int n = (int)(ry / H), yy = (int)(ry - (long)n * H);
-        row = (long)Wtp + ((long)n * (H + 2) + yy + 1) * Wtp + xt;
-    }
+    if (pr >= cvk_wgradp_pad_count(N, H, Wt, Wtp)) return;
+    const long row = cvk_wgradp_pad_row(pr, N, H, Wt, Wtp);
     const f32x4 z = {0.f, 0.f, 0.f, 0.f};
     const size_t ps = (size_t)rows * C;
     for (int x = 0; x < nplanes; ++x)
diff --git a/pytorch-camvid_amd/csrc/wgradp_pads.h b/pytorch-camvid_amd/csrc/wgradp_pads.h
--- /dev/null
+++ b/pytorch-camvid_amd/csrc/wgradp_pads.h
@@ -0,0 +1,25 @@
+#pragma once
+
+__host__ __device__ inline long cvk_wgradp_rows(int N, int H, int Wtp) { return (long)N * (H + 2) * Wtp + 2L * Wtp; }
+
+__host__ __device__ inline long cvk_wgradp_pad_count(int N, int H, int Wt, int Wtp) {
+    return 2L * Wtp + (long)N * 2 * Wtp + (long)N * H * (Wtp - Wt);
+}
+
+__host__ __device__ inline long cvk_wgradp_pad_row(long pr, int N, int H, int Wt, int Wtp) {
+    const long rows = cvk_wgradp_rows(N, H, Wtp);
+    const int padc = Wtp - Wt;
+    const long n_end = 2L * Wtp, n_border = (long)N * 2 * Wtp;
+    if (pr < n_end) return pr < Wtp ? pr : rows - Wtp + (pr - Wtp);
+    if (pr < n_end + n_border) {
+        const long k = pr - n_end;
+        const int n = (int)(k / (2 * Wtp)), rem = (int)(k - (long)n * 2 * Wtp);
+        const int yp = rem < Wtp ? 0 : H + 1, xt = rem < Wtp ? rem : rem - Wtp;
+        return (long)Wtp + ((long)n * (H + 2) + yp) * Wtp + xt;
+    }
+    const long k = pr - n_end - n_border;
+    const long ry = k / padc;
+    const int xt = Wt + (int)(k - ry * padc);
+    const int n = (int)(ry / H), yy = (int)(ry - (long)n * H);
+    return (long)Wtp + ((long)n * (H + 2) + yy + 1) * Wtp + xt;
+}
diff --git a/pytorch-camvid_amd/engine.py b/pytorch-camvid_amd/engine.py
--- a/pytorch-camvid_amd/engine.py
+++ b/pytorch-camvid_amd/engine.py
@@ -526,6 +526,15 @@
         self.wcache_builds = 0
         self.wgrad_side = os.environ.get("CVK_WGRAD_SIDE", WGRAD_SIDE_DEFAULT) != "0"
         self.side_families = WGRAD_SIDE_FAMILIES
+        self.bwd_chain = {"0": False, "1": True, "z": "z", "fin": "fin"}[os.environ.get("CVK_BWD_CHAIN", "z")]
+
+    @property
+    def chain_z(self):
+        return self.bwd_chain in (True, "z")
+
+    @property
+    def chain_fin(self):
+        return self.bwd_chain in (True, "fin")
 
     def side_allowed(self, fold):
         return (self.wgrad_side and not self.bf16 and self.grad_sync is None and self.accumulator is None and fold is None and PROF is None
@@ -729,7 +738,7 @@
 
     def kernel_config(self):
         return (self.wino, self.wino4, self.wino4f, self.wino2d, self.wgradp, self.vplanes, self.thin, self.pool_bnred, self.w2d_split,
-                self.w2tile_cfg)
+                self.w2tile_cfg, self.bwd_chain)
 
     def routes(self, plan, training, need_grad):
         key = (self.kernel_config(), training, need_grad)
```
